# Algolzw/image-restoration-sde

Measured on AMD Instinct MI355X. Metric: restored images/sec at 256x256, 100-step IR-SDE reverse sampler, higher is better.
Workload: dtype f32; 1 GPU; IR-SDE deraining ConditionalUNet nf=64 depth=4, reverse_sde, batch=16/GPU 256x256, T=100 (BASELINE.json configs[1]); compute_dtype=fp32, global_batch=16

## Files before the change

### image_restoration_sde_amd/_lib.py

```python
import ctypes
import os
import subprocess
import threading

_HERE = os.path.dirname(os.path.abspath(__file__))
LIB_PATH = os.environ.get("IRSDE_LIB_PATH") or os.path.join(_HERE, "libirsde_hip.so")
CSRC = os.path.join(_HERE, "csrc")

MODE = {"sde": 0, "ode": 1, "posterior": 2, "dsde_sde": 3, "dsde_ode": 4}
COEF_STRIDE = 12
FLAG_KEEP_ACTIVATIONS = 1
FLAG_NAIVE_CONV = 2
FLAG_NO_WINOGRAD = 4
FLAG_NO_WINOGRAD_F43 = 8
FLAG_UNCOND_FULLATTN = 16
FLAG_BF16 = 32
FLAG_NAF_INTRO_SKIP = 64
FLAG_BF16_ACT = 128
FLAG_NO_FUSED_LN = 256
FLAG_NAF_LENS = 512
FLAG_FP16 = 1024
FLAG_NO_WINOGRAD_FUSED = 2048
FLAG_NO_FUSED_ATTN = 4096
FLAG_NO_NAF_CHAIN = 8192
FLAG_SPLIT_BF16X2 = 16384
FLAG_SPLIT_F16X2 = 32768
FLAG_NAF_STEREO = 65536
FLAG_NAF_UNCOND = 131072
FLAG_UNET_STEREO = 262144
FLAG_F16_ACT = 524288
FLAG_NO_WINO_POLY = 1048576
FLAG_SCAM_STREAM = 2097152
FLAG_NO_SPLIT3 = 4194304
SAMPLE_GRAPH = 1
SAMPLE_PROFILE = 2

SYMBOLS = [
    "irsde_last_error", "irsde_version", "irsde_create", "irsde_create_nafnet", "irsde_destroy", "irsde_num_weights",
    "irsde_weight_name", "irsde_weight_shape", "irsde_load_weight", "irsde_finalize_weights",
    "irsde_set_schedule", "irsde_unet_forward", "irsde_sample", "irsde_sde_step", "irsde_philox_normal",
    "irsde_get_profile", "irsde_debug_tap", "irsde_work_model", "irsde_debug_conv", "irsde_debug_conv_choice", "irsde_debug_conv_features", "irsde_plan_describe", "irsde_bench_conv", "irsde_op_profile", "irsde_debug_split_gemm", "irsde_bench_naf_chain", "irsde_debug_force_subbatches", "irsde_debug_force_chain_groups", "irsde_debug_force_wino_poly", "irsde_debug_force_split3", "irsde_debug_force_split3_blocks", "irsde_debug_scam", "irsde_debug_scam_full",
    "irsde_debug_scam_stream", "irsde_debug_scam_full_stream", "irsde_debug_force_scam_stream",
    "irsde_debug_naf_gate_sca", "irsde_debug_tlsc", "irsde_debug_ln_film", "irsde_debug_naf_lnconv", "irsde_debug_naf_chain", "irsde_debug_naf_chain_split_order",
    "irsde_debug_full_attention16",
    "irsde_eval_metrics", "irsde_tensor2img",
    "irsde_set_lens_info", "irsde_nafnet_set_local_pool", "irsde_create_latent_unet", "irsde_latent_shapes", "irsde_latent_encode", "irsde_latent_decode", "irsde_latent_hidden",
]


class IrsdeLibraryError(RuntimeError):
    pass


class IrsdeError(RuntimeError):
    pass


class Config(ctypes.Structure):
    _fields_ = [("in_nc", ctypes.c_int32), ("out_nc", ctypes.c_int32), ("nf", ctypes.c_int32),
                ("depth", ctypes.c_int32), ("device", ctypes.c_int32), ("flags", ctypes.c_int32)]


class NafConfig(ctypes.Structure):
    _fields_ = [("img_channel", ctypes.c_int32), ("width", ctypes.c_int32), ("middle_blk_num", ctypes.c_int32),
                ("n_enc", ctypes.c_int32), ("enc_blk_nums", ctypes.c_int32 * 8), ("n_dec", ctypes.c_int32),
                ("dec_blk_nums", ctypes.c_int32 * 8), ("device", ctypes.c_int32), ("flags", ctypes.c_int32)]


class LatentConfig(ctypes.Structure):
    _fields_ = [("in_ch", ctypes.c_int32), ("out_ch", ctypes.c_int32), ("ch", ctypes.c_int32), ("n_mult", ctypes.c_int32),
                ("ch_mult", ctypes.c_int32 * 8), ("embed_dim", ctypes.c_int32), ("device", ctypes.c_int32),
                ("flags", ctypes.c_int32)]


_lib = None
_lock = threading.Lock()


PROBES_LIB_PATH = os.path.join(_HERE, "libirsde_hip_probes.so")


def build_library(force=False, verbose=False, probes=True):
    if force:
        subprocess.run(["make", "-C", CSRC, "clean"], check=True, capture_output=not verbose)
    for extra in ([], ["PROBES=1"]) if probes else ([],):
        r = subprocess.run(["make", "-j8", "-C", CSRC] + extra, capture_output=True, text=True)
        if r.returncode != 0:
            raise IrsdeLibraryError("building libirsde_hip%s.so failed:\n" % ("_probes" if extra else "") + r.stdout + r.stderr)
        if verbose:
            print(r.stdout)
    return LIB_PATH


def _declare(lib):
    c = ctypes
    P = c.c_void_p
    lib.irsde_last_error.restype = c.c_char_p
    lib.irsde_last_error.argtypes = []
    lib.irsde_version.restype = c.c_int
    lib.irsde_create.argtypes = [c.POINTER(Config), c.POINTER(P)]
    lib.irsde_create_nafnet.argtypes = [c.POINTER(NafConfig), c.POINTER(P)]
    lib.irsde_destroy.argtypes = [P]
    lib.irsde_destroy.restype = None
    lib.irsde_num_weights.argtypes = [P]
    lib.irsde_weight_name.argtypes = [P, c.c_int]
    lib.irsde_weight_name.restype = c.c_char_p
    lib.irsde_weight_shape.argtypes = [P, c.c_int, c.POINTER(c.c_int64), c.POINTER(c.c_int)]
    lib.irsde_load_weight.argtypes = [P, c.c_char_p, P, c.POINTER(c.c_int64), c.c_int]
    lib.irsde_finalize_weights.argtypes = [P]
    lib.irsde_set_schedule.argtypes = [P, c.c_int, P]
    lib.irsde_unet_forward.argtypes = [P, P, P, c.POINTER(c.c_int64), c.c_int, c.c_int, c.c_int, c.c_int, P, P]
    lib.irsde_sample.argtypes = [P, c.c_int, P, P, P, c.c_uint64, c.c_uint64, c.c_int, c.c_int, c.c_int,
                                 c.c_int, c.c_int, P, P, c.c_int]
    lib.irsde_sde_step.argtypes = [c.c_int, c.c_int, P, P, P, P, P, c.c_uint64, c.c_uint64, c.c_int, c.c_int,
                                   c.c_int, c.c_int, P]
    lib.irsde_philox_normal.argtypes = [P, c.c_int, c.c_int, c.c_int, c.c_uint64, c.c_uint64, P]
    lib.irsde_get_profile.argtypes = [P, c.POINTER(c.c_double)]
    lib.irsde_debug_tap.argtypes = [P, c.c_char_p, P, c.POINTER(c.c_int64)]
    lib.irsde_work_model.argtypes = [P, c.c_int, c.c_int, c.c_int, c.POINTER(c.c_double)]
    lib.irsde_debug_conv.argtypes = [P, c.c_int, P, c.c_int, c.c_int, c.c_int, c.c_int, c.c_int, P, c.c_int, c.c_int,
                                     c.c_int, c.c_int, c.c_int, P, P, c.c_int, c.c_int, P, P, c.c_int, c.c_int, P]
    lib.irsde_debug_conv_choice.argtypes = [c.c_int] * 13 + [c.c_uint] + [c.c_int] * 4 + [c.POINTER(c.c_int), c.c_char_p, c.c_int]
    lib.irsde_debug_conv_features.argtypes = ([P, c.c_int, P, c.c_int] + [c.c_int] * 4 + [P] + [c.c_int] * 7 + [P] * 3 + [P, c.c_int, P, P, P, c.c_int] + [c.c_int] * 6 +
                                              [c.POINTER(c.c_int), P, c.c_char_p, c.c_int, P])
    lib.irsde_plan_describe.argtypes = [P, c.c_int, c.c_int, c.c_int, c.c_char_p, c.c_int]
    lib.irsde_op_profile.argtypes = [P, c.c_char_p, c.c_int]
    lib.irsde_bench_conv.argtypes = [c.c_int] * 11 + [c.POINTER(c.c_double)]
    lib.irsde_bench_naf_chain.argtypes = [c.c_int] * 4 + [c.POINTER(c.c_double)]
    lib.irsde_debug_force_subbatches.argtypes = [c.c_int]
    lib.irsde_debug_force_chain_groups.argtypes = [c.c_int]
    lib.irsde_debug_force_wino_poly.argtypes = [c.c_int]
    lib.irsde_debug_force_split3.argtypes = [c.c_int]
    lib.irsde_debug_force_split3_blocks.argtypes = [c.c_int]
    lib.irsde_debug_scam.argtypes = [P, c.c_int, c.c_int, c.c_int, c.c_int] + [P] * 12 + [P, P]
    lib.irsde_debug_scam_full.argtypes = [P, c.c_int, c.c_int, c.c_int, c.c_int] + [P] * 12 + [P, P]
    lib.irsde_debug_scam_stream.argtypes = [P, c.c_int, c.c_int, c.c_int, c.c_int] + [P] * 12 + [c.c_int, P, P]
    lib.irsde_debug_scam_full_stream.argtypes = [P, c.c_int, c.c_int, c.c_int, c.c_int] + [P] * 12 + [c.c_int, P, P]
    lib.irsde_debug_force_scam_stream.argtypes = [c.c_int]
    lib.irsde_debug_naf_gate_sca.argtypes = [P, c.c_int, c.c_int, c.c_int, c.c_int] + [P] * 8
    lib.irsde_debug_tlsc.argtypes = [P] + [c.c_int] * 6 + [P] * 4
    lib.irsde_debug_ln_film.argtypes = [P, c.c_int64, c.c_int, c.c_int64, P, P, P, c.c_int, P, P]
    lib.irsde_debug_naf_lnconv.argtypes = [c.c_int, P, c.c_int64, c.c_int, c.c_int, c.c_int64, P, P, P, c.c_int, P, P, P, c.c_int, P, P, P, P, P]
    lib.irsde_debug_naf_chain.argtypes = [P, P, c.c_int, c.c_int] + [P] * 16 + [P, c.c_int, c.c_int, P, c.c_int, c.c_int, c.c_int, P]
    lib.irsde_debug_naf_chain_split_order.argtypes = [c.c_int, c.c_int, c.POINTER(c.c_int), c.c_int64]
    lib.irsde_debug_full_attention16.argtypes = [P, c.c_int, c.c_int, P, P]
    lib.irsde_debug_split_gemm.argtypes = [P, P, P, c.c_int, c.c_int, c.c_int, c.c_int, c.c_int, P]
    lib.irsde_eval_metrics.argtypes = [P, P, c.c_int, c.c_int, c.c_int, c.c_int, c.c_int, c.POINTER(c.c_double), P]
    lib.irsde_tensor2img.argtypes = [P, P, c.c_int, c.c_int, c.c_int, c.c_int, P]
    lib.irsde_set_lens_info.argtypes = [P, c.POINTER(c.c_float), c.c_int]
    lib.irsde_nafnet_set_local_pool.argtypes = [P, c.c_int, c.c_int, c.c_int, c.c_int]
    lib.irsde_create_latent_unet.argtypes = [c.POINTER(LatentConfig), c.POINTER(P)]
    lib.irsde_latent_shapes.argtypes = [P, c.c_int, c.c_int, c.POINTER(c.c_int64), c.POINTER(c.c_int64), c.POINTER(c.c_int)]
    lib.irsde_latent_encode.argtypes = [P, P, c.c_int, c.c_int, c.c_int, P, c.POINTER(P), P]
    lib.irsde_latent_decode.argtypes = [P, P, c.POINTER(P), c.c_int, c.c_int, c.c_int, P, P]
    lib.irsde_latent_hidden.argtypes = [P, c.c_int, c.c_int, c.c_int, c.c_int, P, P]
    for name in SYMBOLS:
        getattr(lib, name)
    return lib


def lib():
    global _lib
    with _lock:
        if _lib is None:
            if not os.path.exists(LIB_PATH):
                raise IrsdeLibraryError(
                    "libirsde_hip.so not found at %s — build it with `python -c 'import __graft_entry__ as g; "
                    "g.build()'` or `make -C %s`. There is no CPU/PyTorch fallback for this path." % (LIB_PATH, CSRC))
            try:
                _lib = _declare(ctypes.CDLL(LIB_PATH))
            except OSError as ex:
                raise IrsdeLibraryError("failed to load %s: %s" % (LIB_PATH, ex)) from ex
        return _lib


_probes = None


def probes_lib():
    global _probes
    with _lock:
        if _probes is None:
            if not os.path.exists(PROBES_LIB_PATH):
                raise IrsdeLibraryError("libirsde_hip_probes.so not found at %s — build it with `make -C %s PROBES=1`" % (PROBES_LIB_PATH, CSRC))
            try:
                _probes = _declare(ctypes.CDLL(PROBES_LIB_PATH))
            except OSError as ex:
                raise IrsdeLibraryError("failed to load %s: %s" % (PROBES_LIB_PATH, ex)) from ex
        return _probes


def check(rc, L=None):
    if rc != 0:
        msg = (L or lib()).irsde_last_error()
        raise IrsdeError("libirsde_hip error %d: %s" % (rc, msg.decode() if msg else "?"))


def stream_ptr(torch_stream=None):
    import torch
    s = torch_stream if torch_stream is not None else torch.cuda.current_stream()
    return ctypes.c_void_p(s.cuda_stream)
```

### image_restoration_sde_amd/csrc/common.h

```cpp
#pragma once
#include <hip/hip_runtime.h>
#include <cstdint>
#include <cstdio>
#include <cstdlib>
#include <stdexcept>
#include <string>
#include <vector>
#include "split3_layout.h"

namespace irsde {

struct HipError : std::runtime_error {
    using std::runtime_error::runtime_error;
};
struct HipOutOfMemory : HipError {
    using HipError::HipError;
};

inline int tuning_env_int(const char* name, int dflt) {
    static const bool on = [] { const char* t = getenv("IRSDE_TUNING"); return t && atoi(t) == 1; }();
    if (!on) return dflt;
    const char* v = getenv(name);
    return v ? atoi(v) : dflt;
}

#define IRSDE_HIP_CHECK(expr)                                                                  \
    do {                                                                                       \
        hipError_t _e = (expr);                                                                \
        if (_e != hipSuccess) {                                                                \
            throw ::irsde::HipError(std::string(#expr) + " failed: " + hipGetErrorString(_e) + \
                                    " (" __FILE__ ":" + std::to_string(__LINE__) + ")");       \
        }                                                                                      \
    } while (0)

struct ConvParams {
    const float* in0 = nullptr;
    const float* in1 = nullptr;
    int C0 = 0, C1 = 0;
    int pix0 = 0, pix1 = 0;
    int Hin = 0, Win = 0;
    int in_shift = 0;
    const float* w = nullptr;
    const unsigned short* w_bf = nullptr;
    int f16 = 0;
    const unsigned short* w_pair = nullptr;
    float pair_scale = 1.f;
    int Cout = 0;
    int KH = 1, KW = 1, stride = 1, pad_y = 0, pad_x = 0;
    int B = 0, Ho = 0, Wo = 0;
    float* out = nullptr;
    int out_stride = 0;
    const float* bias = nullptr;
    const float* film = nullptr;
    int film_bstride = 0;
    int silu = 0;
    const float* res = nullptr;
    int res_stride = 0;
    int splits = 1;
    float* partial = nullptr;
    const float* zeros = nullptr;
    const float* ch_scale = nullptr;
    const float* in_scale = nullptr;
    int gate = 0;
    const float* gate_film = nullptr;
    int gate_film_bstride = 0;
    int shuffle = 0;
    int nz = 1;
    long long z_in = 0, z_w = 0, z_out = 0;
    int no_direct_epi = 0;
    int in_bf16 = 0, out_bf16 = 0;
    int in_f16 = 0, out_f16 = 0;
    const float* ln_g = nullptr;
    float ln_eps = 1e-5f;
};

struct WinoParams {
    const float* in0 = nullptr;
    const float* in1 = nullptr;
    int C0 = 0, C1 = 0, Hin = 0, Win = 0, in_shift = 0;
    int B = 0, TH = 0, TW = 0, T = 0;
    int tile = 2;
    float* V = nullptr;
    unsigned short* Vs = nullptr;
    int nplanes = 0;
    int v_f16 = 0;
    float v_scale = 1.f;
    int v_pairs = 0;
    int v_triples = 0;
    const float* M = nullptr;
    int Cout = 0;
    float* out = nullptr;
    int out_stride = 0;
    const float* bias = nullptr;
    const float* film = nullptr;
    int film_bstride = 0;
    int silu = 0;
    const float* res = nullptr;
    int res_stride = 0;
};
void launch_wino_input(const WinoParams& p, hipStream_t s);
struct WinoPolyParams {
    int up = 0;
    const float* in = nullptr;
    int C = 0, Hin = 0, Win = 0;
    int B = 0, TH = 0, TW = 0, T = 0;
    float* V = nullptr;
    unsigned short* Vs = nullptr;
    int thread_writer = 0;
    const float* M = nullptr;
    int Cout = 0, Ho = 0, Wo = 0;
    float* out = nullptr;
    int out_stride = 0;
    const float* bias = nullptr;
};
void launch_wino_poly_input(const WinoPolyParams& p, hipStream_t s);
void launch_wino_poly_output(const WinoPolyParams& p, hipStream_t s);
void wino_poly_transform_weights(const float* w_packed, int Cout, int Cin, float* U, int up);
struct SplitGemmArgs {
    const unsigned short* a = nullptr;
    const unsigned short* b = nullptr;
    float* out = nullptr;
    long long plA = 0, plB = 0, pA = 0, pB = 0, pO = 0;
    int M = 0, N = 0, K = 0, lda = 0, ldc = 0;
    float out_scale = 1.f;
    int n_inner = 1;
    int nblk_n = 0;
};
void gemm_split_global_init();
void launch_gemm_split_pairs(const SplitGemmArgs& a, int ncomp, hipStream_t s, int abl = 0, bool f16 = false);
void launch_split_pairs(const float* in, unsigned short* out, size_t rows, int K, hipStream_t s, bool f16 = false,
                        float scale = 1.0f);
struct Split3Launch {
    enum Abl { FULL = 0, NO_LOADS = 1, NO_MFMA = 3, NO_STORES = 4 };
    enum Tri { RULE, ON, OFF };
    Abl abl = FULL;
    Tri walk = RULE;
    Tri drain = RULE;
};
void launch_gemm_split_triples(const SplitGemmArgs& a, int ncomp, hipStream_t s, const Split3Launch& o = {});
void set_force_split3_blocks(int n);
bool gemm_split_triples_fits(long long M, long long N, long long K, long long ldc);
void launch_split_triples(const float* in, unsigned short* out, int ncomp, size_t rows, int K, hipStream_t s);
void launch_split_planes(const float* in, unsigned short* out, size_t n, size_t plane, int nplanes, hipStream_t s, bool f16 = false,
                         float scale = 1.0f);
void launch_wino_output(const WinoParams& p, hipStream_t s);
void wino_transform_weights(const float* w_packed, int Cout, int Cin, float* U, int tile);
bool wino_fused_eligible(const ConvParams& p);
void wino_fused_pack_weights(const float* U, int Cout, int Cin, float* Uf);
void launch_wino_fused(const ConvParams& p, const float* Uf, hipStream_t s, unsigned long long* dbg = nullptr, int dflags = 0);
int wino_fused_num_blocks(const ConvParams& p);
bool wino_fused64_eligible(const ConvParams& p);
void wino_fused64_pack_weights(const float* U, int Cout, int Cin, float* Uf);
void launch_wino_fused64(const ConvParams& p, const float* Uf, hipStream_t s, int variant = 0);
void wino_fused64_set_debug(unsigned long long* buf);
constexpr float kWinoFused64PairVScale = 0.0625f;
void launch_wino_fused64_split_weights(const float* Uf, unsigned short* out, size_t nfloats, float scale, hipStream_t s);
int wino_fused64_num_blocks(const ConvParams& p);
bool wino_fused64_xcd_nb(const ConvParams& p);
void wino_fused_global_init();
int device_cu_count();
bool wino_fused64t_eligible(const ConvParams& p);
long long wino_fused64t_num_items(const ConvParams& p);
void launch_wino_fused64t(const ConvParams& p, const float* Uf, hipStream_t s, int variant = 0);
void wino_fused64t_set_debug(unsigned long long* buf);
void wino_fused_t_global_init();
void naf_chain_global_init();
void naf_chain_set_debug(unsigned long long* buf);
bool naf_chain_shape_ok(int H, int W, int c);
size_t naf_chain_weight_halves(int nblocks);
size_t naf_chain_vec_floats(int nblocks);
void launch_naf_chain(const float* x, float* out, const unsigned short* w, const float* vecs, int nblocks, int B, const float* film, int film_bstride,
                      int film_off, const float* cam, int cam_bstride, int cam_off, hipStream_t s, int variant = 0);
std::vector<int> naf_chain_split_order(int nblocks, int G);
void naf_chain_build_split_weights(const unsigned short* w1, unsigned short* dst, int nblocks, int G, hipStream_t s);
size_t naf_chain_split_scratch_bytes(int B);
int naf_chain_split_groups(int B, int G);
void launch_naf_chain_split(const float* x, float* out, const unsigned short* wG, const float* vecs, int nblocks, int B, const float* film, int film_bstride,
                            int film_off, const float* cam, int cam_bstride, int cam_off, int G, void* scratch, hipStream_t s);
const unsigned* naf_chain_split_error_flag(const void* scratch, int B);
void naf_chain_split_reset(void* scratch, int B);
void naf_chain_set_sabotage(int on);
void attention_global_init();

double conv_flops(const ConvParams& p);
struct ConvTune {
    enum Tile { TILE_AUTO, TILE_128, TILE_256x128, TILE_256, TILE_128_ONE_PER_CU };
    enum Halo { HALO_AUTO, HALO_OFF, HALO_FORCE_512, HALO_FORCE_256 };
    enum ZLoop { ZLOOP_AUTO, ZLOOP_OFF, ZLOOP_ALL, ZLOOP_PAIRS, ZLOOP_FORCE_1X1 };
    bool rules_off = false;
    Tile tile = TILE_AUTO;
    bool no_buffer_desc = false;
    bool no_direct_epi = false;
    Halo halo = HALO_AUTO;
    ZLoop zloop = ZLOOP_AUTO;
};
struct ConvKnobs {
    int small_bn = 2, small_bn_f32 = 0;
    int pair_tile256 = 1, pair_inscale256 = 0;
    int no_bufa = 0;
    int zloop = -1, zloop_1x1 = -1;
    int zloop_maxnk = 32, zloop_minblk = 1024, zloop_deep = 1, zloop_ragged64 = 2048;
};
const ConvKnobs& conv_knobs_from_env();
struct ConvChoice {
    enum Family { PAIR, NARROW3, ZLOOP_BATCH, ZLOOP_1X1, HALO, IGEMM };
    enum Operand { OP_F32, OP_F32_BUF, OP_BF16, OP_F16 };
    enum Storage { ACT_F32, ACT_BF16, ACT_F16 };
    Family family = IGEMM;
    int BM = 0, BN = 0;
    Operand op = OP_F32;
    Storage act = ACT_F32;
    bool inscale = false;
    int zbatch = 0, zrows = 0;
    unsigned gx = 0, gy = 1, gz = 1;
    int threads = 0, lds = 0;
    int row = -1;
    std::string name() const;
    long long blocks() const { return (long long)gx * gy * gz; }
};
int conv_base_bn(int Cout);
void conv_validate(const ConvParams& p);
ConvChoice conv_choose(const ConvParams& p, const ConvTune& t, const ConvKnobs& k, int cu_count);
int conv_instance_count();
void launch_conv(const ConvParams& p, hipStream_t s, const ConvTune& t = {}, const ConvKnobs* knobs = nullptr, ConvChoice* chosen = nullptr);
void conv_global_init();
void conv_halo_global_init();
bool conv_halo_eligible(const ConvParams& p);
bool conv_halo2_wanted(const ConvParams& p, int force);
void launch_conv_halo(const ConvParams& p, hipStream_t s, int force_halo2 = 0);
void launch_fill_random(float* p, size_t n, unsigned seed, float scale, hipStream_t s);
__device__ __forceinline__ float silu_hw(const float v) {
    return v * __builtin_amdgcn_rcpf(1.0f + __builtin_amdgcn_exp2f(v * -1.44269504088896341f));
}

void launch_f32_to_bf16(const float* in, unsigned short* out, size_t n, hipStream_t s);
void launch_f32_to_f16(const float* in, unsigned short* out, size_t n, hipStream_t s);
void launch_bf16_to_f32(const unsigned short* in, float* out, size_t n, hipStream_t s);
void launch_f16_to_f32(const unsigned short* in, float* out, size_t n, hipStream_t s);
void launch_conv_naive(const ConvParams& p, hipStream_t s);

void launch_layernorm(const float* x, const float* g, const float* res, float* out, int64_t M, int C,
                      float eps, hipStream_t s, bool bf16 = false);
void launch_layernorm_film(const float* x, const float* g, const float* scale, const float* shift, int film_bstride,
                           int64_t pixels_per_image, float* out, int64_t M, int C, float eps, hipStream_t s,
                           bool f16 = false);
int dwgate_tiles(int H, int W, int c);
bool naf_lnconv_ok(int c, int Cout, long long M);
void launch_naf_pwconv(const float* x, const float* in_scale, int64_t pixels_per_image, const unsigned short* w16, const float* bias, const float* ch_scale,
                       const float* res, float* out, int64_t M, int c, int Cout, hipStream_t s, bool f16 = false);
void naf_lnconv_global_init();
void launch_naf_lnconv(const float* x, const float* g, const float* fscale, const float* fshift, int film_bstride, int64_t pixels_per_image,
                       const unsigned short* w16, const float* bias, float* out, int64_t M, int c, int Cout, int gate, const float* gate_film,
                       int gate_film_bstride, hipStream_t s, bool f16 = false);
void launch_dwconv_gate(const float* u, const float* w, const float* bias, float* out, float* partial, int B, int H, int W,
                        int c, hipStream_t s, bool f16 = false);
void launch_sca(const float* partial, int ntiles, const float* W, const float* bias, float* mean, float* s_out, int B,
                int c, int HW, hipStream_t s);
void launch_sca_mean(const float* partial, int ntiles, float* mean, int B, int c, int HW, hipStream_t s);
void tlsc_check_shape(int B, int h, int w, int c, int k1, int k2);
void launch_tlsc_pool(const float* gated, float* rowsum, float* pooled, int B, int h, int w, int c, int k1, int k2, hipStream_t s);
void launch_tlsc_scale(float* gated, const float* scale, int B, int h, int w, int c, int k1, int k2, hipStream_t s);
void launch_row_gate(const float* in, float* out, int rows, int h, hipStream_t s);

struct AttnWorkspace {
    float* pmax = nullptr;
    float* pctx = nullptr;
    float* psum = nullptr;
    float* ctx = nullptr;
    int nch = 0;
};
int attn_num_chunks(int N, int B);
void launch_linear_attention(const float* qkv, float* out, int B, int N, const AttnWorkspace& ws, hipStream_t s,
                             bool bf16 = false);

void launch_attention_kv_context(const float* xn, const float* wkv, int B, int N, int C, const AttnWorkspace& ws, hipStream_t s,
                                 const float* ln_g = nullptr, float ln_eps = 1e-5f, const unsigned short* wkv_pair = nullptr,
                                 float w_inv_scale = 1.f, int op16 = 0, bool act_bf16 = false);
void launch_attention_q_out(const float* q, float* out, int B, int N, const AttnWorkspace& ws, hipStream_t s);
void launch_attention_q_out_fused(const float* xn, const float* x, const float* wq, const float* wout, const float* bias,
                                  const float* g2, float* y, int B, int N, int C, float eps, const AttnWorkspace& ws, hipStream_t s,
                                  const float* ln_g = nullptr, const unsigned short* wq_pair = nullptr, const unsigned short* wout_pair = nullptr,
                                  float wq_inv = 1.f, float wout_inv = 1.f, int op16 = 0, bool act_bf16 = false);

void scam_check_shape(int H, int W, int c, bool any_width = false);
void launch_scam_prologue(const float* x, const float* g_l, const float* g_r, float* xs2, int B, int H, int W, int c, hipStream_t s);
void launch_scam_core(const float* qv, float* F, int B, int H, int W, int c, hipStream_t s);
void launch_scam_epilogue(const float* x, const float* F, const float* beta, const float* gamma, float* out, int B, int H, int W, int c, hipStream_t s);
void scam_pack_proj(const float* w1, const float* b1, const float* w2, const float* b2, int c, std::vector<float>& w, std::vector<float>& bias);
constexpr int kScamFullMaxW = 1024;
constexpr int kScamFullMaxC = 2048;
void scam_full_check_shape(int H, int W, int c, bool any_width = false);
void launch_scam_full_prologue(const float* x, const float* g_l, const float* g_r, float* x2, int B, int H, int W, int c, hipStream_t s);
void launch_scam_full_core(const float* qv, float* F, int B, int H, int W, int c, hipStream_t s);
void launch_scam_full_epilogue(float* x, const float* F, const float* beta, const float* gamma, int B, int H, int W, int c, hipStream_t s);
constexpr int kScamMaxWs = 512;
constexpr int kScamStreamMaxBlockW = 512;
bool scam_stream_block_ok(int block_w);
void launch_scam_stream_core(const float* qv, float* F, int B, int Hs, int Ws, int c, int block_w, hipStream_t s);
void launch_stereo_prep(const float* xt, const float* cond, float* x0, int B, int ic, int P, int H, int W, int Hp, int Wp, hipStream_t s);
void launch_stereo_pack_pred(const float* in, float* out, int B, int ic, int Hp, int Wp, int in_stride, int out_stride, hipStream_t s);
void launch_stereo_unet_prep(const float* xt, const float* cond, float* x0, int B, int ic, int P, int H, int W, int Hp, int Wp, hipStream_t s);
void launch_stereo_unet_pack_pred(const float* in, const float* xt, float* out, int B, int ic, int H, int W, int Hp, int Wp, int in_stride, int out_stride,
                                  hipStream_t s);

void launch_full_attention(const float* qkv, float* out, int B, int N, hipStream_t s);
void launch_full_attention16(const unsigned short* qkv, unsigned short* out, int B, int N, hipStream_t s);

void launch_prep_input(const float* xt, const float* cond, float* x0, int B, int in_nc, int H, int W, int Hp, int Wp,
                       hipStream_t s, int reflect = 1);

enum Act { ACT_NONE = 0, ACT_SILU = 1, ACT_GELU = 2 };
void launch_sinusoid(const float* tvals, const float* freqs, float* out, int rows, int half, hipStream_t s);
void launch_row_linear(const float* in, int in_stride, const float* W, const float* b, float* out, int out_stride,
                       int rows, int in_dim, int out_dim, int act_in, int act_out, hipStream_t s);

struct StepState {
    int t;
    int t_next;
    int pad0, pad1;
    float coef[12];
};
void launch_step_begin(StepState* st, const float* film_table, int film_row, float* film_cur,
                       const float* coef_table, hipStream_t s);
void launch_set_step(StepState* st, int t_next, hipStream_t s);

struct SampleCtl {
    int mode;
    int pad;
    const float* noise;
    long long noise_tstride;
    unsigned long long seed;
    unsigned long long image_offset;
};
void launch_set_ctl(SampleCtl* ctl, int mode, const float* noise, long long noise_tstride, unsigned long long seed,
                    unsigned long long image_offset, hipStream_t s);

void launch_unpack_pred(const float* pred, float* out, int B, int C, int H, int W, int Hp, int Wp, int stride, hipStream_t s);
void launch_add(const float* a, const float* b, float* out, size_t n, hipStream_t s);
void launch_nchw_to_nhwc_pad(const float* in, float* out, int B, int C, int H, int W, int Hp, int Wp, int Cp, int reflect,
                             hipStream_t s);
void launch_nhwc_to_nchw(const float* in, float* out, int B, int C, int H, int W, hipStream_t s, bool bf16 = false, bool f16 = false);

struct UpdateParams {
    float* x;
    const float* mu;
    const float* pred;
    int64_t sb, sc, sy, sx;
    const float* noise;
    int64_t noise_tstride;
    const StepState* st;
    const SampleCtl* ctl;
    int t_imm;
    float coef_imm[12];
    int mode;
    int B, C, H, W;
    uint64_t seed;
    uint64_t image_offset;
    int batch0;
};
void launch_sde_update(const UpdateParams& p, hipStream_t s);
void launch_philox_normal(float* out, int B, int CHW, int t, uint64_t seed, uint64_t image_offset, hipStream_t s);

void eval_metrics(const float* out, const float* gt, int B, int C, int H, int W, int crop, double* sums_host, hipStream_t s);
void tensor2img_u8(const float* in, unsigned char* out, int B, int C, int H, int W, hipStream_t s);

}
```

### image_restoration_sde_amd/csrc/engine_debug.hip

```cpp
#include "engine.h"
#include "../../include/irsde_hip_debug.h"

using namespace irsde;

namespace irsde {
namespace {

struct Scratch {
    hipStream_t s;
    std::vector<void*> bufs;
    explicit Scratch(hipStream_t s_) : s(s_) {}
    ~Scratch() {
        (void)hipStreamSynchronize(s);
        for (void* p : bufs) (void)hipFree(p);
    }
    Scratch(const Scratch&) = delete;
    Scratch& operator=(const Scratch&) = delete;
    template <class T> T* alloc(size_t n) {
        void* p = nullptr;
        IRSDE_HIP_CHECK(hipMalloc(&p, n * sizeof(T)));
        bufs.push_back(p);
        return static_cast<T*>(p);
    }
    float* upload(const float* host, size_t n) {
        float* d = alloc<float>(n);
        IRSDE_HIP_CHECK(hipMemcpy(d, host, n * sizeof(float), hipMemcpyHostToDevice));
        return d;
    }
    float* upload(const std::vector<float>& v) { return upload(v.data(), v.size()); }
};
struct OwnedStream {
    hipStream_t s = nullptr;
    explicit OwnedStream(unsigned flags) { IRSDE_HIP_CHECK(hipStreamCreateWithFlags(&s, flags)); }
    ~OwnedStream() { (void)hipStreamDestroy(s); }
    OwnedStream(const OwnedStream&) = delete;
    OwnedStream& operator=(const OwnedStream&) = delete;
};
struct EventPair {
    hipEvent_t e0 = nullptr, e1 = nullptr;
    EventPair() {
        IRSDE_HIP_CHECK(hipEventCreate(&e0));
        IRSDE_HIP_CHECK(hipEventCreate(&e1));
    }
    ~EventPair() {
        if (e0) (void)hipEventDestroy(e0);
        if (e1) (void)hipEventDestroy(e1);
    }
    EventPair(const EventPair&) = delete;
    EventPair& operator=(const EventPair&) = delete;
};
template <class Run>
double time_launches(hipStream_t s, int iters, Run&& run) {
    EventPair ev;
    IRSDE_HIP_CHECK(hipEventRecord(ev.e0, s));
    for (int i = 0; i < iters; ++i) run();
    IRSDE_HIP_CHECK(hipEventRecord(ev.e1, s));
    IRSDE_HIP_CHECK(hipStreamSynchronize(s));
    float ms = 0.f;
    IRSDE_HIP_CHECK(hipEventElapsedTime(&ms, ev.e0, ev.e1));
    return ms / iters;
}


ConvTune conv_tune_from_code(int code) {
    ConvTune t;
    t.rules_off = code != 0;
    switch (code) {
        case 3: t.tile = ConvTune::TILE_256x128; break;
        case 50: t.tile = ConvTune::TILE_256; break;
        case 5: t.tile = ConvTune::TILE_128_ONE_PER_CU; break;
        case 6: t.no_buffer_desc = true; break;
        case 7: t.no_direct_epi = true; break;
        case 60: t.tile = ConvTune::TILE_256; t.halo = ConvTune::HALO_OFF; break;
        case 61: t.tile = ConvTune::TILE_128; t.halo = ConvTune::HALO_OFF; break;
        case 64: t.halo = ConvTune::HALO_FORCE_512; break;
        case 65: t.halo = ConvTune::HALO_FORCE_256; break;
        case 70: t.zloop = ConvTune::ZLOOP_OFF; break;
        case 71: t.zloop = ConvTune::ZLOOP_ALL; break;
        case 72: t.zloop = ConvTune::ZLOOP_PAIRS; break;
        case 73: t.zloop = ConvTune::ZLOOP_FORCE_1X1; break;
        default: break;
    }
    return t;
}

Split3Launch split3_launch_twin(int twin, int abl = 0) {
    Split3Launch o;
    o.abl = static_cast<Split3Launch::Abl>(abl);
    o.walk = twin == 0 ? Split3Launch::RULE : twin == 1 ? Split3Launch::OFF : Split3Launch::ON;
    o.drain = twin == 0 ? Split3Launch::RULE : twin == 1 ? Split3Launch::OFF : Split3Launch::ON;
    return o;
}

enum class Operand { F32, BF16, F16 };

enum class ConvPath {
    Direct,
    Valu,
    WinoF2,
    WinoF4,
    Poly,
    PolyTriples,
    F4Triples,
    F4Pairs,
    DirectPair,
    Fused32,
    Fused64,
    Fused64Pair,
    Fused64T,
};
struct DebugConvRow {
    int code;
    ConvPath path;
    Operand op;
    bool act_bf16;
    int tune;
    int variant;
    bool up;
    bool thread_writer;
};
constexpr DebugConvRow direct(int code, Operand op, bool act_bf16, int tune) { return {code, ConvPath::Direct, op, act_bf16, tune, 0, false, false}; }
constexpr DebugConvRow on_path(int code, ConvPath path, Operand op = Operand::F32) { return {code, path, op, false, 0, 0, false, false}; }
constexpr DebugConvRow wino(int code, ConvPath path, int tune) { return {code, path, Operand::F32, false, tune, 0, false, false}; }
constexpr DebugConvRow poly(int code, ConvPath path, bool up, bool thread_writer = false) { return {code, path, Operand::F32, false, 0, 0, up, thread_writer}; }
constexpr DebugConvRow fused(int code, ConvPath path, int variant) { return {code, path, Operand::F32, false, 0, variant, false, false}; }
constexpr DebugConvRow kDebugConv[] = {
    direct(0, Operand::F32, false, 0),
    on_path(1, ConvPath::Valu),
    wino(2, ConvPath::WinoF2, 0), wino(12, ConvPath::WinoF2, 71), wino(22, ConvPath::WinoF2, 72),
    wino(3, ConvPath::WinoF4, 0), wino(13, ConvPath::WinoF4, 71), wino(23, ConvPath::WinoF4, 72),
    poly(24, ConvPath::Poly, false), poly(25, ConvPath::Poly, true),
    poly(26, ConvPath::PolyTriples, false), poly(27, ConvPath::PolyTriples, true), poly(28, ConvPath::PolyTriples, true, true),
    on_path(48, ConvPath::F4Triples),
    on_path(44, ConvPath::F4Pairs, Operand::F16), on_path(45, ConvPath::F4Pairs, Operand::BF16),
    on_path(46, ConvPath::DirectPair, Operand::F16), on_path(47, ConvPath::DirectPair, Operand::BF16),
    on_path(33, ConvPath::Fused32),
    fused(34, ConvPath::Fused64, 0), fused(36, ConvPath::Fused64, 64), fused(55, ConvPath::Fused64, 20),
    fused(35, ConvPath::Fused64Pair, 4), fused(37, ConvPath::Fused64Pair, 4 + 64), fused(56, ConvPath::Fused64Pair, 24),
    fused(62, ConvPath::Fused64T, 0), fused(63, ConvPath::Fused64T, 64),
    direct(4, Operand::BF16, false, 0), direct(160, Operand::BF16, false, 60), direct(161, Operand::BF16, false, 61), direct(162, Operand::BF16, false, 64),
    direct(163, Operand::BF16, false, 65),
    direct(5, Operand::F16, false, 0), direct(165, Operand::F16, false, 61), direct(166, Operand::F16, false, 64), direct(167, Operand::F16, false, 65),
    direct(204, Operand::BF16, true, 0), direct(260, Operand::BF16, true, 60), direct(261, Operand::BF16, true, 61), direct(262, Operand::BF16, true, 64),
    direct(263, Operand::BF16, true, 65),
    direct(100, Operand::F32, false, 0), direct(103, Operand::F32, false, 3), direct(105, Operand::F32, false, 5), direct(106, Operand::F32, false, 6),
    direct(107, Operand::F32, false, 7), direct(150, Operand::F32, false, 50), direct(170, Operand::F32, false, 70), direct(171, Operand::F32, false, 71),
    direct(172, Operand::F32, false, 72), direct(173, Operand::F32, false, 73),
};

enum class BenchKind {
    Conv,
    Fused32,
    Fused32Stamps,
    Wino3,
    Wino3Gemm,
    Fused64,
    Fused64Stamps,
    Fused64T,
    Fused64TStamps,
    PairGemm,
    TripleGemm,
};
struct BenchRow {
    int lo, hi;
    BenchKind kind;
    int arg;
    Operand op;
    bool pair;
    bool act_bf16;
};
constexpr BenchRow bench(int lo, int hi, BenchKind kind, int arg, Operand op = Operand::F32, bool pair = false, bool act_bf16 = false) {
    return {lo, hi, kind, arg, op, pair, act_bf16};
}
constexpr BenchRow kBenchConv[] = {
    bench(0, 0, BenchKind::Conv, 0), bench(3, 3, BenchKind::Conv, 3), bench(5, 7, BenchKind::Conv, 5), bench(50, 50, BenchKind::Conv, 50),
    bench(70, 73, BenchKind::Conv, 70),
    bench(60, 61, BenchKind::Conv, 60, Operand::BF16),
    bench(62, 62, BenchKind::Conv, 0, Operand::BF16),
    bench(63, 63, BenchKind::Conv, 0, Operand::BF16, false, true),
    bench(64, 65, BenchKind::Conv, 64, Operand::BF16),
    bench(66, 67, BenchKind::Conv, 64, Operand::BF16, false, true),
    bench(480, 480, BenchKind::Conv, 0, Operand::F16, true), bench(481, 481, BenchKind::Conv, 0, Operand::BF16, true),
    bench(482, 482, BenchKind::Conv, 61, Operand::F16, true),
    bench(80, 80, BenchKind::Fused32, 0),
    bench(83, 82 + 255, BenchKind::Fused32, 1),
    bench(82, 82, BenchKind::Fused32Stamps, 0),
    bench(81, 81, BenchKind::Wino3, 0), bench(421, 421, BenchKind::Wino3Gemm, 0),
    bench(430, 432, BenchKind::Fused64, 20),
    bench(434, 434, BenchKind::Fused64, 24, Operand::F16),
    bench(435, 435, BenchKind::Fused64Stamps, 25), bench(2004, 2004, BenchKind::Fused64Stamps, 25),
    bench(2001, 2002, BenchKind::Fused64Stamps, 28),
    bench(460, 462, BenchKind::Fused64T, 0),
    bench(467, 469, BenchKind::Fused64T, 6),
    bench(465, 465, BenchKind::Fused64TStamps, 5),
    bench(4650, 4653, BenchKind::Fused64TStamps, 12),
    bench(472, 476, BenchKind::PairGemm, 0),
    bench(490, 504, BenchKind::TripleGemm, 0),
};

template <class Row, size_t N, class Lo, class Hi>
constexpr bool codes_disjoint(const Row (&rows)[N], Lo lo, Hi hi) {
    for (size_t i = 0; i < N; ++i)
        for (size_t j = 0; j < N; ++j)
            if (i != j && lo(rows[i]) <= hi(rows[j]) && lo(rows[j]) <= hi(rows[i])) return false;
    return true;
}
constexpr int row_code(const DebugConvRow& r) { return r.code; }
constexpr int row_lo(const BenchRow& r) { return r.lo; }
constexpr int row_hi(const BenchRow& r) { return r.hi; }
static_assert(codes_disjoint(kDebugConv, row_code, row_code), "irsde_debug_conv: a selector code has two rows");
static_assert(codes_disjoint(kBenchConv, row_lo, row_hi), "irsde_bench_conv: a variant has two rows");

const DebugConvRow& debug_conv_lookup(int code) {
    for (const DebugConvRow& r : kDebugConv)
        if (r.code == code) return r;
    throw HipError("debug_conv: unknown selector code " + std::to_string(code));
}
struct BenchSel {
    const BenchRow& row;
    int arg;
};
BenchSel bench_conv_lookup(int code) {
    for (const BenchRow& r : kBenchConv)
        if (code >= r.lo && code <= r.hi) return {r, r.arg + (code - r.lo)};
    throw HipError("bench_conv: unknown variant " + std::to_string(code));
}

SplitGemmArgs split_gemm_args(const unsigned short* a, const unsigned short* b, float* C, int M, int N, int K, size_t pA, size_t pB) {
    SplitGemmArgs g;
    g.a = a; g.b = b; g.out = C;
    g.pA = (long long)pA; g.pB = (long long)pB; g.pO = (long long)M * N;
    g.M = M; g.N = N; g.K = K; g.lda = K; g.ldc = N;
    return g;
}
SplitGemmArgs split_triples(Scratch& mem, const float* A, const float* Bm, float* C, int M, int N, int K, int ncomp, hipStream_t s) {
    const size_t ea = split3_comp_elems((size_t)M, (size_t)K), eb = split3_comp_elems((size_t)N, (size_t)K);
    unsigned short *ta = mem.alloc<unsigned short>(ea * ncomp), *tb = mem.alloc<unsigned short>(eb * ncomp);
    launch_split_triples(A, ta, ncomp, (size_t)M, K, s);
    launch_split_triples(Bm, tb, ncomp, (size_t)N, K, s);
    return split_gemm_args(ta, tb, C, M, N, K, ea, eb);
}
SplitGemmArgs split_pairs(Scratch& mem, const float* A, const float* Bm, float* C, int M, int N, int K, int ncomp, hipStream_t s, bool f16 = false, float sa = 1.f,
                          float sb = 1.f) {
    unsigned short *pa = mem.alloc<unsigned short>((size_t)2 * ncomp * M * K), *pb = mem.alloc<unsigned short>((size_t)2 * ncomp * N * K);
    launch_split_pairs(A, pa, (size_t)ncomp * M, K, s, f16, sa);
    launch_split_pairs(Bm, pb, (size_t)ncomp * N, K, s, f16, sb);
    SplitGemmArgs g = split_gemm_args(pa, pb, C, M, N, K, (size_t)M * K, (size_t)N * K);
    g.out_scale = 1.0f / (sa * sb);
    return g;
}

void write_choice_line(const ConvChoice& c, char* out, int out_len) {
    snprintf(out, (size_t)out_len, "name=%s family=%d tile=%dx%d op=%d act=%d inscale=%d zbatch=%d zrows=%d grid=%ux%ux%u threads=%d lds=%d row=%d of %d",
             c.name().c_str(), (int)c.family, c.BM, c.BN, (int)c.op, (int)c.act, (int)c.inscale, c.zbatch, c.zrows, c.gx, c.gy, c.gz, c.threads, c.lds, c.row,
             conv_instance_count());
}

struct ScamHookArgs {
    const float* x;
    float* out;
    const float *norm_l_g, *norm_r_g, *l_proj1_w, *l_proj1_b, *r_proj1_w, *r_proj1_b, *l_proj2_w, *l_proj2_b, *r_proj2_w, *r_proj2_b, *beta, *gamma;
};
struct ScamHookDev {
    float *gl, *gr, *beta, *gamma;
    float *in2, *qv, *F;
    size_t vsz;
};
template <class ShapeCheck, class Prologue, class Tail>
void scam_hook(const ScamHookArgs& a, int B, int Hs, int Ws, int C, void* stream, ShapeCheck check_shape, Prologue prologue, Tail tail) {
    if (!a.x || !a.out || !a.norm_l_g || !a.norm_r_g || !a.l_proj1_w || !a.l_proj1_b || !a.r_proj1_w || !a.r_proj1_b || !a.l_proj2_w || !a.l_proj2_b ||
        !a.r_proj2_w || !a.r_proj2_b || !a.beta || !a.gamma)
        throw HipError("null argument");
    check_shape();
    hipStream_t s = reinterpret_cast<hipStream_t>(stream);
    conv_global_init();
    std::vector<float> wl, bl, wr, br;
    scam_pack_proj(a.l_proj1_w, a.l_proj1_b, a.l_proj2_w, a.l_proj2_b, C, wl, bl);
    scam_pack_proj(a.r_proj1_w, a.r_proj1_b, a.r_proj2_w, a.r_proj2_b, C, wr, br);
    Scratch mem(s);
    auto up = [&](const float* h, size_t n) {
        float* d = mem.alloc<float>(std::max<size_t>(n, 16));
        if (h) IRSDE_HIP_CHECK(hipMemcpy(d, h, n * 4, hipMemcpyHostToDevice));
        return d;
    };
    ScamHookDev d;
    d.gl = up(a.norm_l_g, C); d.gr = up(a.norm_r_g, C); d.beta = up(a.beta, C); d.gamma = up(a.gamma, C);
    float *dwl = up(wl.data(), wl.size()), *dbl = up(bl.data(), bl.size()), *dwr = up(wr.data(), wr.size()), *dbr = up(br.data(), br.size());
    d.vsz = (size_t)B * Hs * Ws * 2 * C;
    d.in2 = up(nullptr, 2 * d.vsz); d.qv = up(nullptr, 2 * d.vsz); d.F = up(nullptr, d.vsz);
    float* dz = up(nullptr, 256);
    IRSDE_HIP_CHECK(hipMemset(dz, 0, 1024));
    prologue(d, s);
    for (int v = 0; v < 2; ++v) {
        ConvParams p;
        p.in0 = d.in2 + v * d.vsz; p.C0 = 2 * C; p.pix0 = 2 * C;
        p.Hin = Hs; p.Win = Ws;
        p.w = v ? dwr : dwl; p.Cout = 2 * C; p.KH = p.KW = 1; p.stride = 1;
        p.B = B; p.Ho = Hs; p.Wo = Ws;
        p.out = d.qv + v * d.vsz; p.out_stride = 2 * C;
        p.bias = v ? dbr : dbl;
        p.zeros = dz;
        launch_conv(p, s);
    }
    tail(d, s);
    IRSDE_HIP_CHECK(hipStreamSynchronize(s));
}

}
}

extern "C" {

int irsde_debug_scam(const float* x, int B, int H, int W, int C, const float* norm_l_g, const float* norm_r_g, const float* l_proj1_w,
                     const float* l_proj1_b, const float* r_proj1_w, const float* r_proj1_b, const float* l_proj2_w, const float* l_proj2_b,
                     const float* r_proj2_w, const float* r_proj2_b, const float* beta, const float* gamma, float* out, void* stream) {
    return guard([&] {
        scam_hook(
            {x, out, norm_l_g, norm_r_g, l_proj1_w, l_proj1_b, r_proj1_w, r_proj1_b, l_proj2_w, l_proj2_b, r_proj2_w, r_proj2_b, beta, gamma}, B, H / 4, W / 4, C, stream,
            [&] {
                if (B < 1) throw HipError("debug_scam: bad shape");
                scam_check_shape(H, W, C);
            },
            [&](const ScamHookDev& d, hipStream_t s) { launch_scam_prologue(x, d.gl, d.gr, d.in2, B, H, W, C, s); },
            [&](const ScamHookDev& d, hipStream_t s) {
                launch_scam_core(d.qv, d.F, B, H, W, C, s);
                launch_scam_epilogue(x, d.F, d.beta, d.gamma, out, B, H, W, C, s);
            });
    });
}

int irsde_debug_scam_full(const float* x, int B, int H, int W, int C, const float* norm_l_g, const float* norm_r_g, const float* l_proj1_w,
                          const float* l_proj1_b, const float* r_proj1_w, const float* r_proj1_b, const float* l_proj2_w, const float* l_proj2_b,
                          const float* r_proj2_w, const float* r_proj2_b, const float* beta, const float* gamma, float* out, void* stream) {
    return guard([&] {
        scam_hook(
            {x, out, norm_l_g, norm_r_g, l_proj1_w, l_proj1_b, r_proj1_w, r_proj1_b, l_proj2_w, l_proj2_b, r_proj2_w, r_proj2_b, beta, gamma}, B, H, W, C, stream,
            [&] {
                if (B < 1 || (long long)B * H > 65535) throw HipError("debug_scam_full: bad shape");
                scam_full_check_shape(H, W, C);
            },
            [&](const ScamHookDev& d, hipStream_t s) { launch_scam_full_prologue(x, d.gl, d.gr, d.in2, B, H, W, C, s); },
            [&](const ScamHookDev& d, hipStream_t s) {
                launch_scam_full_core(d.qv, d.F, B, H, W, C, s);
                if (out != x) IRSDE_HIP_CHECK(hipMemcpyAsync(out, x, d.vsz * sizeof(float), hipMemcpyDeviceToDevice, s));
                launch_scam_full_epilogue(out, d.F, d.beta, d.gamma, B, H, W, C, s);
            });
    });
}

int irsde_debug_scam_stream(const float* x, int B, int H, int W, int C, const float* norm_l_g, const float* norm_r_g, const float* l_proj1_w,
                            const float* l_proj1_b, const float* r_proj1_w, const float* r_proj1_b, const float* l_proj2_w, const float* l_proj2_b,
                            const float* r_proj2_w, const float* r_proj2_b, const float* beta, const float* gamma, int block_w, float* out, void* stream) {
    return guard([&] {
        scam_hook(
            {x, out, norm_l_g, norm_r_g, l_proj1_w, l_proj1_b, r_proj1_w, r_proj1_b, l_proj2_w, l_proj2_b, r_proj2_w, r_proj2_b, beta, gamma}, B, H / 4, W / 4, C, stream,
            [&] {
                if (B < 1 || (long long)B * (H / 4) > 65535) throw HipError("debug_scam_stream: bad shape");
                if (block_w != 0 && !scam_stream_block_ok(block_w)) throw HipError("debug_scam_stream: block_w must be 0 or a multiple of 16 in [16, 512]");
                scam_check_shape(H, W, C, true);
            },
            [&](const ScamHookDev& d, hipStream_t s) { launch_scam_prologue(x, d.gl, d.gr, d.in2, B, H, W, C, s); },
            [&](const ScamHookDev& d, hipStream_t s) {
                launch_scam_stream_core(d.qv, d.F, B, H / 4, W / 4, C, block_w, s);
                launch_scam_epilogue(x, d.F, d.beta, d.gamma, out, B, H, W, C, s);
            });
    });
}

int irsde_debug_scam_full_stream(const float* x, int B, int H, int W, int C, const float* norm_l_g, const float* norm_r_g, const float* l_proj1_w,
                                 const float* l_proj1_b, const float* r_proj1_w, const float* r_proj1_b, const float* l_proj2_w, const float* l_proj2_b,
                                 const float* r_proj2_w, const float* r_proj2_b, const float* beta, const float* gamma, int block_w, float* out,
                                 void* stream) {
    return guard([&] {
        scam_hook(
            {x, out, norm_l_g, norm_r_g, l_proj1_w, l_proj1_b, r_proj1_w, r_proj1_b, l_proj2_w, l_proj2_b, r_proj2_w, r_proj2_b, beta, gamma}, B, H, W, C, stream,
            [&] {
                if (B < 1 || (long long)B * H > 65535) throw HipError("debug_scam_full_stream: bad shape");
                if (block_w != 0 && !scam_stream_block_ok(block_w)) throw HipError("debug_scam_full_stream: block_w must be 0 or a multiple of 16 in [16, 512]");
                scam_full_check_shape(H, W, C, true);
            },
            [&](const ScamHookDev& d, hipStream_t s) { launch_scam_full_prologue(x, d.gl, d.gr, d.in2, B, H, W, C, s); },
            [&](const ScamHookDev& d, hipStream_t s) {
                launch_scam_stream_core(d.qv, d.F, B, H, W, C, block_w, s);
                if (out != x) IRSDE_HIP_CHECK(hipMemcpyAsync(out, x, d.vsz * sizeof(float), hipMemcpyDeviceToDevice, s));
                launch_scam_full_epilogue(out, d.F, d.beta, d.gamma, B, H, W, C, s);
            });
    });
}

int irsde_debug_force_scam_stream(int block_w) {
    if (block_w != 0 && !scam_stream_block_ok(block_w)) return guard([&] { throw HipError("debug_force_scam_stream: block_w must be 0 or a multiple of 16 in [16, 512]"); });
    set_force_scam_stream(block_w);
    return IRSDE_OK;
}

int irsde_debug_naf_gate_sca(const float* u, int B, int H, int W, int c, const float* conv2_w, const float* conv2_b, const float* sca_w, const float* sca_b,
                             float* gated_out, float* mean_out, float* s_out, void* stream) {
    return guard([&] {
        if (!u || !conv2_w || !conv2_b || !sca_w || !sca_b || !gated_out || !s_out) throw HipError("null argument");
        if (B < 1 || B > 65535 || H < 1 || W < 1 || c < 4 || c % 4 || (long long)H * W >= (1ll << 31)) throw HipError("debug_naf_gate_sca: bad shape");
        hipStream_t s = reinterpret_cast<hipStream_t>(stream);
        conv_global_init();
        Scratch mem(s);
        float *dw = mem.upload(pack_dwconv_taps(conv2_w, 2 * c)), *db = mem.upload(conv2_b, (size_t)2 * c);
        float *dsw = mem.upload(sca_w, (size_t)c * c), *dsb = mem.upload(sca_b, c);
        const int nt = dwgate_tiles(H, W, c);
        float *partial = mem.alloc<float>((size_t)B * nt * c), *mean = mem.alloc<float>((size_t)B * c);
        launch_dwconv_gate(u, dw, db, gated_out, partial, B, H, W, c, s);
        launch_sca(partial, nt, dsw, dsb, mean, s_out, B, c, H * W, s);
        if (mean_out) launch_sca_mean(partial, nt, mean_out, B, c, H * W, s);
        IRSDE_HIP_CHECK(hipStreamSynchronize(s));
    });
}

int irsde_debug_tlsc(const float* g, int B, int h, int w, int c, int k1, int k2, float* pooled_out, const float* scale_map, float* scaled_out, void* stream) {
    return guard([&] {
        if (!g || !pooled_out || !scale_map || !scaled_out) throw HipError("null argument");
        tlsc_check_shape(B, h, w, c, k1, k2);
        hipStream_t s = reinterpret_cast<hipStream_t>(stream);
        conv_global_init();
        Scratch mem(s);
        float* rowsum = mem.alloc<float>((size_t)B * h * (w - k2 + 1) * c);
        launch_tlsc_pool(g, rowsum, pooled_out, B, h, w, c, k1, k2, s);
        IRSDE_HIP_CHECK(hipMemcpyAsync(scaled_out, g, (size_t)B * h * w * c * sizeof(float), hipMemcpyDeviceToDevice, s));
        launch_tlsc_scale(scaled_out, scale_map, B, h, w, c, k1, k2, s);
        IRSDE_HIP_CHECK(hipStreamSynchronize(s));
    });
}

int irsde_debug_ln_film(const float* x, long long M, int C, long long ppi, const float* g, const float* fscale, const float* fshift, int film_bstride,
                        float* out, void* stream) {
    return guard([&] {
        if (!x || !g || !fscale || !fshift || !out) throw HipError("null argument");
        if (M < 1 || ppi < 1 || C < 4 || C % 4 || C > 2048 || film_bstride < 0 || film_bstride % 4) throw HipError("debug_ln_film: bad shape");
        hipStream_t s = reinterpret_cast<hipStream_t>(stream);
        conv_global_init();
        Scratch mem(s);
        float* dg = mem.upload(g, C);
        launch_layernorm_film(x, dg, fscale, fshift, film_bstride, ppi, out, M, C, 1e-5f, s);
        IRSDE_HIP_CHECK(hipStreamSynchronize(s));
    });
}

int irsde_debug_full_attention16(const void* qkv_bf16, int B, int N, void* out_bf16, void* stream) {
    return guard([&] {
        if (!qkv_bf16 || !out_bf16) throw HipError("null argument");
        hipStream_t s = reinterpret_cast<hipStream_t>(stream);
        launch_full_attention16(static_cast<const unsigned short*>(qkv_bf16), static_cast<unsigned short*>(out_bf16), B, N, s);
        IRSDE_HIP_CHECK(hipStreamSynchronize(s));
    });
}

int irsde_debug_naf_lnconv(int mode, const float* x, long long M, int c, int Cout, long long ppi, const float* g, const float* fscale, const float* fshift,
                           int film_bstride, const float* w, const float* bias, const float* gate_film, int gate_film_bstride, const float* in_scale,
                           const float* ch_scale, const float* res, float* out, void* stream) {
    return guard([&] {
        if (mode < 0 || mode > 3) throw HipError("debug_naf_lnconv: mode must be 0 .. 3");
        if (!x || !w || !bias || !out) throw HipError("null argument");
        if (!naf_lnconv_ok(c, Cout, M) || ppi < 1) throw HipError("debug_naf_lnconv: bad shape");
        const bool ln = mode <= 1;
        if (ln && (!g || !fscale || !fshift || film_bstride < 0 || film_bstride % 4)) throw HipError("debug_naf_lnconv: modes 0 / 1 need g and the FiLM rows");
        if (mode == 1 && gate_film && gate_film_bstride < 0) throw HipError("debug_naf_lnconv: bad lens FiLM stride");
        if (!ln && (!ch_scale || !res || (mode == 2 && !in_scale))) throw HipError("debug_naf_lnconv: modes 2 / 3 need ch_scale and res, mode 2 in_scale");
        hipStream_t s = reinterpret_cast<hipStream_t>(stream);
        conv_global_init();
        std::vector<float> pw, pb;
        pack_conv_rows(w, bias, Cout, c, 1, 1, mode == 1 ? naf_gate_perm(Cout / 2) : std::vector<int>(), pw, pb);
        Scratch mem(s);
        float *dwf = mem.upload(pw), *dbias = mem.upload(pb);
        unsigned short* w16 = mem.alloc<unsigned short>(pw.size());
        launch_f32_to_f16(dwf, w16, pw.size(), s);
        if (ln) {
            float* dg = mem.upload(g, c);
            launch_naf_lnconv(x, dg, fscale, fshift, film_bstride, ppi, w16, dbias, out, M, c, Cout, mode, mode == 1 ? gate_film : nullptr,
                              mode == 1 && gate_film ? gate_film_bstride : 0, s);
        } else {
            float* dcs = mem.upload(ch_scale, Cout);
            launch_naf_pwconv(x, mode == 2 ? in_scale : nullptr, ppi, w16, dbias, dcs, res, out, M, c, Cout, s);
        }
        IRSDE_HIP_CHECK(hipStreamSynchronize(s));
    });
}

int irsde_debug_naf_chain(const float* x, float* out, int B, int nblocks, const float* norm1_g, const float* conv1_w, const float* conv1_b, const float* conv2_w,
                          const float* conv2_b, const float* sca_w, const float* sca_b, const float* conv3_w, const float* conv3_b, const float* beta,
                          const float* norm2_g, const float* conv4_w, const float* conv4_b, const float* conv5_w, const float* conv5_b, const float* gamma,
                          const float* film, int film_bstride, int film_off, const float* cam, int cam_bstride, int cam_off, int groups, void* stream) {
    return guard([&] {
        if (!x || !out || !norm1_g || !conv1_w || !conv1_b || !conv2_w || !conv2_b || !sca_w || !sca_b || !conv3_w || !conv3_b || !beta || !norm2_g || !conv4_w ||
            !conv4_b || !conv5_w || !conv5_b || !gamma || !film)
            throw HipError("null argument");
        if (B < 1 || B > 65535 || nblocks < 1 || nblocks > 64) throw HipError("debug_naf_chain: bad B or nblocks");
        if (groups != 1 && groups != 2 && groups != 4) throw HipError("debug_naf_chain: groups must be 1, 2 or 4");
        if (film_bstride < 0 || film_bstride % 4 || film_off < 0 || film_off % 4) throw HipError("debug_naf_chain: bad FiLM stride / offset");
        if (cam && (cam_bstride < 0 || cam_bstride % 4 || cam_off < 0 || cam_off % 4)) throw HipError("debug_naf_chain: bad lens FiLM stride / offset");
        hipStream_t s = reinterpret_cast<hipStream_t>(stream);
        conv_global_init();
        if (groups > 1 && naf_chain_split_groups(B, groups) > device_cu_count())
            throw HipError("debug_naf_chain: more work-groups than compute units (they must be co-resident)");
        constexpr size_t C = 512;
        std::vector<NafChainHostW> blocks(nblocks);
        for (int i = 0; i < nblocks; ++i) {
            NafChainHostW& b = blocks[i];
            const size_t k = (size_t)i;
            b.norm1_g = norm1_g + k * C; b.conv1_w = conv1_w + k * 2 * C * C; b.conv1_b = conv1_b + k * 2 * C;
            b.conv2_w = conv2_w + k * 18 * C; b.conv2_b = conv2_b + k * 2 * C;
            b.sca_w = sca_w + k * C * C; b.sca_b = sca_b + k * C;
            b.conv3_w = conv3_w + k * C * C; b.conv3_b = conv3_b + k * C; b.beta = beta + k * C;
            b.norm2_g = norm2_g + k * C; b.conv4_w = conv4_w + k * 2 * C * C; b.conv4_b = conv4_b + k * 2 * C;
            b.conv5_w = conv5_w + k * C * C; b.conv5_b = conv5_b + k * C; b.gamma = gamma + k * C;
        }
        std::vector<unsigned short> w;
        std::vector<float> vecs;
        pack_naf_chain_host(blocks, w, vecs);
        Scratch mem(s);
        unsigned short* dw = mem.alloc<unsigned short>(w.size());
        IRSDE_HIP_CHECK(hipMemcpy(dw, w.data(), w.size() * 2, hipMemcpyHostToDevice));
        float* dvec = mem.upload(vecs);
        if (groups == 1) {
            launch_naf_chain(x, out, dw, dvec, nblocks, B, film, film_bstride, film_off, cam, cam ? cam_bstride : 0, cam ? cam_off : 0, s, 0);
            IRSDE_HIP_CHECK(hipStreamSynchronize(s));
            return;
        }
        unsigned short* dwg = mem.alloc<unsigned short>(w.size());
        naf_chain_build_split_weights(dw, dwg, nblocks, groups, s);
        const size_t sb = naf_chain_split_scratch_bytes(B);
        char* dscratch = mem.alloc<char>(sb);
        IRSDE_HIP_CHECK(hipMemset(dscratch, 0, sb));
        launch_naf_chain_split(x, out, dwg, dvec, nblocks, B, film, film_bstride, film_off, cam, cam ? cam_bstride : 0, cam ? cam_off : 0, groups, dscratch, s);
        IRSDE_HIP_CHECK(hipStreamSynchronize(s));
        std::vector<unsigned> state((size_t)4 * B + 1);
        IRSDE_HIP_CHECK(hipMemcpy(state.data(), naf_chain_split_error_flag(dscratch, B) - 4 * B, state.size() * 4, hipMemcpyDeviceToHost));
        if (state[(size_t)4 * B]) throw HipError("debug_naf_chain: the split kernel's groups were not co-resident (spin timeout)");
        for (size_t i = 0; i < (size_t)4 * B; ++i)
            if (state[i]) throw HipError("debug_naf_chain: the split kernel left a barrier counter non-zero");
    });
}

int irsde_debug_naf_chain_split_order(int nblocks, int groups, int* order_out, long long n) {
    return guard([&] {
        if (!order_out || nblocks < 1 || nblocks > 64) throw HipError("debug_naf_chain_split_order: bad argument");
        const std::vector<int> order = naf_chain_split_order(nblocks, groups);
        if ((long long)order.size() != n) throw HipError("debug_naf_chain_split_order: the order has " + std::to_string(order.size()) + " entries");
        std::copy(order.begin(), order.end(), order_out);
    });
}

int irsde_debug_conv(const float* in0, int C0, const float* in1, int C1, int B, int Hin, int Win, int in_shift,
                     const float* w_oihw, int Cout, int KH, int KW, int stride, int pad, const float* bias,
                     const float* film, int film_bstride, int silu, const float* res, float* out, int naive,
                     int splits, void* stream) {
    return guard([&] {
        if (!in0 || !w_oihw || !out) throw HipError("null argument");
        const DebugConvRow& r = debug_conv_lookup(naive);
        hipStream_t s = reinterpret_cast<hipStream_t>(stream);
        conv_global_init();
        const int Cin = C0 + C1;
        std::vector<float> pk((size_t)Cout * KH * KW * Cin);
        for (int o = 0; o < Cout; ++o)
            for (int i = 0; i < Cin; ++i)
                for (int ky = 0; ky < KH; ++ky)
                    for (int kx = 0; kx < KW; ++kx)
                        pk[(((size_t)o * KH + ky) * KW + kx) * Cin + i] = w_oihw[(((size_t)o * Cin + i) * KH + ky) * KW + kx];
        Scratch mem(s);
        float* dw = mem.upload(pk);
        float* db = bias ? mem.upload(bias, Cout) : nullptr;
        ConvParams p;
        p.in0 = in0; p.C0 = C0; p.pix0 = C0; p.in1 = in1; p.C1 = C1; p.pix1 = C1;
        p.Hin = Hin; p.Win = Win; p.in_shift = in_shift;
        p.w = dw; p.Cout = Cout; p.KH = KH; p.KW = KW; p.stride = stride; p.pad_y = pad; p.pad_x = pad;
        p.B = B;
        p.Ho = ((Hin << in_shift) + 2 * pad - KH) / stride + 1;
        p.Wo = ((Win << in_shift) + 2 * pad - KW) / stride + 1;
        p.out = out; p.out_stride = Cout; p.bias = db; p.film = film; p.film_bstride = film_bstride; p.silu = silu;
        p.res = res; p.res_stride = Cout;
        float* dz = mem.alloc<float>(256);
        IRSDE_HIP_CHECK(hipMemset(dz, 0, 1024));
        p.zeros = dz;
        if (splits > 1 && r.path != ConvPath::Valu && r.path != ConvPath::WinoF2 && r.path != ConvPath::WinoF4) {
            p.splits = splits;
            p.partial = mem.alloc<float>((size_t)splits * B * p.Ho * p.Wo * Cout);
        }
        auto wino_weights = [&](int tile) {
            std::vector<float> U((size_t)(tile + 2) * (tile + 2) * Cout * Cin);
            wino_transform_weights(pk.data(), Cout, Cin, U.data(), tile);
            return U;
        };
        auto wino_tiles = [&](int tile) { return (long long)B * (p.Ho / tile) * (p.Wo / tile); };
        auto alloc_M = [&](int ncomp, long long T) { return mem.alloc<float>((size_t)ncomp * T * Cout); };
        auto poly_plan = [&](const char* refusal, float*& dU) {
            if (!(r.up ? wino_poly_up_shape(p) : wino_poly_down_shape(p)) || !wino_poly_eligible(p) || splits > 1) throw HipError(refusal);
            std::vector<float> U((size_t)100 * Cout * Cin);
            wino_poly_transform_weights(pk.data(), Cout, Cin, U.data(), r.up);
            dU = mem.upload(U);
            return make_wino_poly(p, dU, nullptr, nullptr);
        };
        switch (r.path) {
        case ConvPath::PolyTriples: {
            float* dU = nullptr;
            WinoPolyPlan wp = poly_plan("debug_conv: selectors 26 / 27 / 28 run what 24 / 25 run (single source, channels a multiple of 32, bias only)", dU);
            if (!gemm_split_triples_fits(wp.T, Cout, wp.K, Cout)) throw HipError("debug_conv: shape not eligible for the three-piece GEMM");
            unsigned short* dUt = mem.alloc<unsigned short>((size_t)wp.ncomp * split3_comp_elems((size_t)Cout, (size_t)wp.K));
            unsigned short* dVt = mem.alloc<unsigned short>((size_t)wp.ncomp * split3_comp_elems((size_t)wp.T, (size_t)wp.K));
            float* dM = alloc_M(wp.ncomp, wp.T);
            launch_split_triples(dU, dUt, wp.ncomp, (size_t)Cout, wp.K, s);
            wp = make_wino_poly(p, dU, nullptr, dM);
            const SplitGemmArgs sg = make_wino_poly_triples(wp, Cout, dUt, dVt, dM);
            wp.in.thread_writer = r.thread_writer;
            launch_wino_poly_input(wp.in, s);
            launch_gemm_split_triples(sg, wp.ncomp, s);
            launch_wino_poly_output(wp.out, s);
            break;
        }
        case ConvPath::Poly: {
            float* dU = nullptr;
            WinoPolyPlan wp = poly_plan(r.up ? "debug_conv: selector 25 runs a 3x3 stride-1 pad-1 convolution with in_shift = 1 (single source, channels a multiple of 32, bias only)"
                                             : "debug_conv: selector 24 runs a 4x4 stride-2 pad-1 convolution (single source, channels a multiple of 32, bias only)", dU);
            float* dV = mem.alloc<float>((size_t)wp.ncomp * wp.T * wp.K);
            wp = make_wino_poly(p, dU, dV, alloc_M(wp.ncomp, wp.T));
            launch_wino_poly_input(wp.in, s);
            launch_conv(wp.gemm, s);
            launch_wino_poly_output(wp.out, s);
            break;
        }
        case ConvPath::F4Triples: {
            if (!wino_shape_ok(p, 4) || Cin % 32) throw HipError("debug_conv: shape not eligible for the three-piece GEMM");
            const std::vector<float> U = wino_weights(4);
            const long long T = wino_tiles(4);
            if (!gemm_split_triples_fits(T, Cout, Cin, Cout)) throw HipError("debug_conv: shape not eligible for the three-piece GEMM");
            float* dU = mem.upload(U);
            unsigned short* dUt = mem.alloc<unsigned short>((size_t)36 * split3_comp_elems((size_t)Cout, (size_t)Cin));
            unsigned short* dVt = mem.alloc<unsigned short>((size_t)36 * split3_comp_elems((size_t)T, (size_t)Cin));
            launch_split_triples(dU, dUt, 36, (size_t)Cout, Cin, s);
            const WinoSplitPlan sp = make_wino_triples(p, dUt, dVt, alloc_M(36, T));
            launch_wino_input(sp.in, s);
            launch_gemm_split_triples(sp.gemm, 36, s);
            launch_wino_output(sp.out, s);
            break;
        }
        case ConvPath::F4Pairs: {
            const bool f16 = r.op == Operand::F16;
            if (!wino_shape_ok(p, 4) || Cin % 32) throw HipError("debug_conv: shape not eligible for the pair GEMM");
            std::vector<float> U = wino_weights(4);
            const float us = f16 ? pow2_scale_into_512(U.data(), U.size()) : 1.f;
            const long long T = wino_tiles(4);
            float* dU = mem.upload(U);
            unsigned short* dUp = mem.alloc<unsigned short>(2 * U.size());
            unsigned short* dVp = mem.alloc<unsigned short>((size_t)36 * T * Cin * 2);
            launch_split_pairs(dU, dUp, (size_t)36 * Cout, Cin, s, f16, us);
            const WinoSplitPlan sp = make_wino_pairs(p, dUp, dVp, alloc_M(36, T), f16, us);
            launch_wino_input(sp.in, s);
            launch_gemm_split_pairs(sp.gemm, 36, s, 0, f16);
            launch_wino_output(sp.out, s);
            break;
        }
        case ConvPath::Fused64Pair: {
            if (!wino_fused64_eligible(p)) throw HipError("debug_conv: shape not eligible for the fused Winograd kernel");
            std::vector<float> U = wino_weights(4), Uf(U.size());
            wino_fused64_pack_weights(U.data(), Cout, Cin, Uf.data());
            const float usc = pow2_scale_into_512(U.data(), U.size());
            float* dUf = mem.upload(Uf);
            unsigned short* dUp = mem.alloc<unsigned short>(2 * Uf.size());
            launch_wino_fused64_split_weights(dUf, dUp, Uf.size(), usc, s);
            p.pair_scale = 1.0f / (kWinoFused64PairVScale * usc);
            launch_wino_fused64(p, reinterpret_cast<const float*>(dUp), s, r.variant);
            break;
        }
        case ConvPath::Fused32:
        case ConvPath::Fused64:
        case ConvPath::Fused64T: {
            const bool f32k = r.path == ConvPath::Fused32;
            if (f32k ? !wino_fused_eligible(p) : !wino_fused64_eligible(p)) throw HipError("debug_conv: shape not eligible for the fused Winograd kernel");
            const std::vector<float> U = wino_weights(4);
            std::vector<float> Uf(U.size());
            if (f32k) wino_fused_pack_weights(U.data(), Cout, Cin, Uf.data());
            else wino_fused64_pack_weights(U.data(), Cout, Cin, Uf.data());
            float* dUf = mem.upload(Uf);
            if (r.path == ConvPath::Fused64T) {
                if (!wino_fused64t_eligible(p)) throw HipError("debug_conv: shape not eligible for the two-tile-group fused Winograd kernel");
                launch_wino_fused64t(p, dUf, s, r.variant);
            } else if (f32k) {
                launch_wino_fused(p, dUf, s);
            } else {
                launch_wino_fused64(p, dUf, s, r.variant);
            }
            break;
        }
        case ConvPath::WinoF2:
        case ConvPath::WinoF4: {
            const int tile = r.path == ConvPath::WinoF2 ? 2 : 4, ncomp = (tile + 2) * (tile + 2);
            if (!wino_shape_ok(p, tile)) throw HipError("debug_conv: shape not eligible for Winograd");
            const std::vector<float> U = wino_weights(tile);
            const long long T = wino_tiles(tile);
            float* dU = mem.upload(U);
            float* dV = mem.alloc<float>((size_t)ncomp * T * Cin);
            const WinoPlan wp = make_wino(p, dU, dV, alloc_M(ncomp, T), tile);
            launch_wino_input(wp.in, s);
            launch_conv(wp.gemm, s, conv_tune_from_code(r.tune));
            launch_wino_output(wp.out, s);
            break;
        }
        case ConvPath::DirectPair: {
            const bool f16 = r.op == Operand::F16;
            const float sc = f16 ? pow2_scale_into_512(pk.data(), pk.size()) : 1.f;
            unsigned short* dwp = mem.alloc<unsigned short>(2 * pk.size());
            launch_split_pairs(dw, dwp, (size_t)Cout, KH * KW * (C0 + C1), s, f16, sc);
            p.w_pair = dwp; p.pair_scale = 1.0f / sc; p.f16 = f16 ? 1 : 0;
            launch_conv(p, s);
            break;
        }
        case ConvPath::Valu:
            launch_conv_naive(p, s);
            break;
        case ConvPath::Direct: {
            unsigned short* ao = nullptr;
            if (r.op != Operand::F32) {
                unsigned short* d16 = mem.alloc<unsigned short>(pk.size());
                if (r.op == Operand::F16) launch_f32_to_f16(dw, d16, pk.size(), s);
                else launch_f32_to_bf16(dw, d16, pk.size(), s);
                p.w_bf = d16;
                p.f16 = r.op == Operand::F16 ? 1 : 0;
            }
            const size_t npix_in = (size_t)B * Hin * Win, nout = (size_t)B * p.Ho * p.Wo * Cout;
            if (r.act_bf16) {
                auto to_bf = [&](const float* src, size_t n) {
                    unsigned short* d = mem.alloc<unsigned short>(n + 32);
                    launch_f32_to_bf16(src, d, n, s);
                    return reinterpret_cast<const float*>(d);
                };
                p.in0 = to_bf(in0, npix_in * C0);
                if (in1) p.in1 = to_bf(in1, npix_in * C1);
                if (res) p.res = to_bf(res, nout);
                ao = mem.alloc<unsigned short>(nout + 32);
                p.out = reinterpret_cast<float*>(ao);
                p.in_bf16 = p.out_bf16 = 1;
            }
            launch_conv(p, s, conv_tune_from_code(r.tune));
            if (r.act_bf16) launch_bf16_to_f32(ao, out, nout, s);
            break;
        }
        }
        IRSDE_HIP_CHECK(hipStreamSynchronize(s));
    });
}

int irsde_debug_conv_choice(int B, int Hin, int Win, int C0, int C1, int Cout, int K, int stride, int pad, int in_shift, int operand, int storage, int pair,
                            unsigned features, int splits, int nz, int tune, int cu_count, const int* knobs, char* out, int out_len) {
    return guard([&] {
        if (!out || out_len < 1 || K < 1 || stride < 1 || cu_count < 1 || operand < 0 || operand > 2 || storage < 0 || storage > 2 || (pair && operand == 0))
            throw HipError("debug_conv_choice: bad argument");
        static const float dummy[4] = {};
        float* const some = const_cast<float*>(dummy);
        auto bit = [&](int i) { return (features >> i & 1u) ? some : nullptr; };
        ConvParams p;
        p.in0 = some; p.C0 = C0; p.pix0 = C0; p.in1 = C1 ? some : nullptr; p.C1 = C1; p.pix1 = C1;
        p.Hin = Hin; p.Win = Win; p.in_shift = in_shift;
        p.w = some; p.Cout = Cout; p.KH = K; p.KW = K; p.stride = stride; p.pad_y = pad; p.pad_x = pad;
        p.B = B;
        p.Ho = ((Hin << in_shift) + 2 * pad - K) / stride + 1;
        p.Wo = ((Win << in_shift) + 2 * pad - K) / stride + 1;
        p.out = some; p.out_stride = Cout; p.res_stride = Cout; p.zeros = some;
        p.bias = bit(0); p.film = bit(1); p.silu = bit(2) != nullptr; p.res = bit(3); p.in_scale = bit(4); p.ch_scale = bit(5);
        p.gate = bit(6) != nullptr; p.shuffle = bit(7) != nullptr; p.ln_g = bit(8);
        if (pair) p.w_pair = reinterpret_cast<const unsigned short*>(some);
        else if (operand) p.w_bf = reinterpret_cast<const unsigned short*>(some);
        p.f16 = operand == 2;
        p.in_bf16 = p.out_bf16 = storage == 1;
        p.in_f16 = p.out_f16 = storage == 2;
        p.nz = nz;
        if (splits > 1) { p.splits = splits; p.partial = some; }
        ConvKnobs k;
        static_assert(sizeof(ConvKnobs) == 11 * sizeof(int), "the hook's knob array is ConvKnobs, field by field");
        if (knobs) memcpy(&k, knobs, sizeof k);
        conv_validate(p);
        const ConvChoice c = conv_choose(p, conv_tune_from_code(tune), k, cu_count);
        const bool tabled = c.family != ConvChoice::NARROW3 && c.family != ConvChoice::HALO;
        if (tabled && c.row < 0) throw HipError("launch_conv: no kernel instance " + c.name());
        write_choice_line(c, out, out_len);
    });
}

int irsde_debug_conv_features(const float* in0, int C0, const float* in1, int C1, int B, int Hin, int Win, int in_shift, const float* w_oihw, int Cout, int K,
                              int stride, int pad, int operand, int storage, int pair, const float* bias, const float* ch_scale, const float* ln_g,
                              const float* film, int film_bstride, const float* res, const float* in_scale, const float* gate_film, int gate_film_bstride,
                              int silu, int gate, int shuffle, int nz, int splits, int tune, const int* knobs, float* out, char* choice, int choice_len,
                              void* stream) {
    return guard([&] {
        if (!in0 || !w_oihw || !out || !choice || choice_len < 1) throw HipError("null argument");
        if (B < 1 || Hin < 1 || Win < 1 || C0 < 1 || C1 < 0 || (C1 > 0) != (in1 != nullptr) || Cout < 1 || K < 1 || stride < 1 || pad < 0 || in_shift < 0 || in_shift > 1 ||
            operand < 0 || operand > 2 || storage < 0 || storage > 2 || (pair && operand == 0) || nz < 1 || splits < 1 || film_bstride < 0 || gate_film_bstride < 0)
            throw HipError("debug_conv_features: bad argument");
        if ((gate && shuffle) || (gate && (Cout % 4 || res)) || (shuffle && Cout % 4) || (gate_film && !gate) || ((gate || shuffle) && film))
            throw HipError("debug_conv_features: gate needs Cout % 4 == 0 and takes no residual, shuffle needs Cout % 4 == 0, gate_film goes with gate, film with neither");
        if (nz > 1 && (B != 1 || Hin != 1 || K != 1 || stride != 1 || pad || in_shift || C1 || storage))
            throw HipError("debug_conv_features: nz > 1 is a stack of 1x1 GEMMs: B = 1, Hin = 1, K = 1, one fp32 source");
        const int Ho = ((Hin << in_shift) + 2 * pad - K) / stride + 1, Wo = ((Win << in_shift) + 2 * pad - K) / stride + 1;
        if (Ho < 1 || Wo < 1) throw HipError("debug_conv_features: empty output");
        hipStream_t s = reinterpret_cast<hipStream_t>(stream);
        conv_global_init();
        const int Cin = C0 + C1;
        const std::vector<int> perm = gate ? naf_gate_perm(Cout / 2) : shuffle ? naf_shuffle_perm(Cout) : std::vector<int>();
        const size_t wz = (size_t)Cout * K * K * Cin;
        std::vector<float> pk(wz * nz), pb, one, oneb;
        for (int z = 0; z < nz; ++z) {
            pack_conv_rows(w_oihw + z * wz, z == 0 ? bias : nullptr, Cout, Cin, K, K, perm, one, z == 0 ? pb : oneb);
            std::copy(one.begin(), one.end(), pk.begin() + z * wz);
        }
        Scratch mem(s);
        float* dw = mem.upload(pk);
        ConvParams p;
        p.in0 = in0; p.C0 = C0; p.pix0 = C0; p.in1 = in1; p.C1 = C1; p.pix1 = C1;
        p.Hin = Hin; p.Win = Win; p.in_shift = in_shift;
        p.w = dw; p.Cout = Cout; p.KH = K; p.KW = K; p.stride = stride; p.pad_y = pad; p.pad_x = pad;
        p.B = B; p.Ho = Ho; p.Wo = Wo;
        const int ostride = gate ? Cout / 2 : shuffle ? Cout / 4 : Cout;
        const size_t npix_in = (size_t)B * Hin * Win * nz, M = (size_t)B * Ho * Wo, nout = M * nz * (gate ? Cout / 2 : Cout);
        p.out = out; p.out_stride = ostride; p.res = res; p.res_stride = ostride;
        if (bias) p.bias = mem.upload(pb);
        if (ch_scale) {
            std::vector<float> cs(Cout);
            for (int o = 0; o < Cout; ++o) cs[o] = ch_scale[perm.empty() ? o : perm[o]];
            p.ch_scale = mem.upload(cs);
        }
        if (ln_g) p.ln_g = mem.upload(ln_g, Cout);
        p.film = film; p.film_bstride = film_bstride; p.silu = silu; p.in_scale = in_scale;
        p.gate = gate ? 1 : 0; p.gate_film = gate_film; p.gate_film_bstride = gate_film ? gate_film_bstride : 0; p.shuffle = shuffle ? 1 : 0;
        p.nz = nz;
        if (nz > 1) { p.z_in = (long long)Win * C0; p.z_w = (long long)Cout * C0; p.z_out = (long long)Win * Cout; }
        float* dz = mem.alloc<float>(256);
        IRSDE_HIP_CHECK(hipMemset(dz, 0, 1024));
        p.zeros = dz;
        if (splits > 1) {
            p.splits = splits;
            p.partial = mem.alloc<float>((size_t)splits * M * Cout);
        }
        const bool f16 = operand == 2;
        unsigned short *w16 = nullptr, *a0 = nullptr, *a1 = nullptr, *ar = nullptr, *ao = nullptr;
        float wsc = 1.f;
        if (pair) {
            wsc = f16 ? pow2_scale_into_512(pk.data(), pk.size()) : 1.f;
            w16 = mem.alloc<unsigned short>(2 * pk.size());
            p.w_pair = w16; p.pair_scale = 1.0f / wsc;
        } else if (operand) {
            w16 = mem.alloc<unsigned short>(pk.size());
            p.w_bf = w16;
        }
        p.f16 = f16 ? 1 : 0;
        if (storage) {
            a0 = mem.alloc<unsigned short>(npix_in * C0);
            p.in0 = reinterpret_cast<const float*>(a0);
            if (in1) { a1 = mem.alloc<unsigned short>(npix_in * C1); p.in1 = reinterpret_cast<const float*>(a1); }
            if (res) { ar = mem.alloc<unsigned short>(nout); p.res = reinterpret_cast<const float*>(ar); }
            ao = mem.alloc<unsigned short>(nout);
            p.out = reinterpret_cast<float*>(ao);
            p.in_bf16 = p.out_bf16 = storage == 1;
            p.in_f16 = p.out_f16 = storage == 2;
        }
        ConvKnobs k;
        static_assert(sizeof(ConvKnobs) == 11 * sizeof(int), "the hook's knob array is ConvKnobs, field by field");
        if (knobs) memcpy(&k, knobs, sizeof k);
        conv_validate(p);
        auto narrow = [&](const float* src, unsigned short* dst, size_t n) {
            if (storage == 2) launch_f32_to_f16(src, dst, n, s);
            else launch_f32_to_bf16(src, dst, n, s);
        };
        if (pair) launch_split_pairs(dw, w16, (size_t)Cout * nz, K * K * Cin, s, f16, wsc);
        else if (operand == 2) launch_f32_to_f16(dw, w16, pk.size(), s);
        else if (operand == 1) launch_f32_to_bf16(dw, w16, pk.size(), s);
        if (storage) {
            narrow(in0, a0, npix_in * C0);
            if (in1) narrow(in1, a1, npix_in * C1);
            if (res) narrow(res, ar, nout);
            IRSDE_HIP_CHECK(hipMemsetAsync(ao, 0xFF, nout * 2, s));
        }
        ConvChoice c;
        launch_conv(p, s, conv_tune_from_code(tune), knobs ? &k : nullptr, &c);
        if (storage == 2) launch_f16_to_f32(ao, out, nout, s);
        else if (storage == 1) launch_bf16_to_f32(ao, out, nout, s);
        IRSDE_HIP_CHECK(hipStreamSynchronize(s));
        write_choice_line(c, choice, choice_len);
    });
}

int irsde_debug_split_gemm(const float* A, const float* Bm, float* C, int M, int N, int K, int ncomp, int nplanes, void* stream) {
    return guard([&] {
        const int twin3 = nplanes == 43 ? 0 : nplanes == 45 ? 1 : nplanes == 47 ? 2 : -1;
        if (twin3 < 0 && nplanes != 42 && nplanes != 44) throw HipError("debug_split_gemm: nplanes must be 42, 43, 44, 45 or 47");
        hipStream_t s = reinterpret_cast<hipStream_t>(stream);
        conv_global_init();
        Scratch mem(s);
        if (twin3 >= 0) {
            if (!gemm_split_triples_fits(M, N, K, N)) throw HipError("debug_split_gemm: shape not eligible for the three-piece GEMM");
            launch_gemm_split_triples(split_triples(mem, A, Bm, C, M, N, K, ncomp, s), ncomp, s, split3_launch_twin(twin3));
        } else {
            const bool f16 = nplanes == 44;
            launch_gemm_split_pairs(split_pairs(mem, A, Bm, C, M, N, K, ncomp, s, f16, f16 ? 1.0f / 16.0f : 1.f, f16 ? 64.0f : 1.f), ncomp, s, 0, f16);
        }
        IRSDE_HIP_CHECK(hipStreamSynchronize(s));
    });
}

int irsde_debug_force_chain_groups(int g) {
    set_force_chain_groups(g == 1 || g == 2 || g == 4 ? g : 0);
    return IRSDE_OK;
}

int irsde_debug_force_split3(int mode) {
    set_force_split3(mode >= 0 && mode <= 2 ? mode : -1);
    return IRSDE_OK;
}

int irsde_debug_force_split3_blocks(int n) {
    if (n >= 0 && n < 8) return guard([&] { throw HipError("debug_force_split3_blocks: n must be at least 8 (one block per XCD), or negative for the default"); });
    set_force_split3_blocks(n);
    return IRSDE_OK;
}

int irsde_debug_force_wino_poly(int mode) {
    set_force_wino_poly(mode >= 0 && mode <= 2 ? mode : -1);
    return IRSDE_OK;
}

int irsde_debug_force_subbatches(int n) {
    set_force_subbatches(n < 0 ? 0 : n);
    return IRSDE_OK;
}

int irsde_bench_naf_chain(int variant, int nblocks, int B, int iters, double* ms_out) {
    return guard([&] {
        if (!ms_out || nblocks < 1 || nblocks > 64 || B < 1 || iters < 1) throw HipError("bench_naf_chain: bad argument");
        const int G = variant == 22 ? 2 : (variant == 24 || variant == 25 || variant == 26) ? 4 : 1;
#ifdef IRSDE_PROBES
        if (variant != 0 && variant != 1 && variant != 11 && G == 1) throw HipError("bench_naf_chain: bad variant");
#else
        if (variant != 0 && variant != 1 && G == 1) throw HipError("bench_naf_chain: variant 11 is a measurement twin (make PROBES=1)");
#endif
        conv_global_init();
        OwnedStream stream(hipStreamDefault);
        hipStream_t s = stream.s;
        Scratch mem(s);
        const size_t nx = (size_t)B * 64 * 512, nw = naf_chain_weight_halves(nblocks), nv = naf_chain_vec_floats(nblocks);
        float *dx = mem.alloc<float>(nx), *dout = mem.alloc<float>(nx), *dvec = mem.alloc<float>(nv), *dfilm = mem.alloc<float>((size_t)nblocks * 2048);
        unsigned short* dw = mem.alloc<unsigned short>(nw);
        const size_t chunk = (size_t)64 << 20;
        float* dwf = mem.alloc<float>(chunk);
        launch_fill_random(dx, nx, 1, 1.0f, s);
        launch_fill_random(dvec, nv, 2, 0.1f, s);
        launch_fill_random(dfilm, (size_t)nblocks * 2048, 3, 0.1f, s);
        for (size_t o = 0; o < nw; o += chunk) {
            const size_t n = std::min(chunk, nw - o);
            launch_fill_random(dwf, n, 4 + (unsigned)(o / chunk), 0.04f, s);
            launch_f32_to_f16(dwf, dw + o, n, s);
        }
        unsigned short* dwg = nullptr;
        void* dscratch = nullptr;
        if (G > 1) {
            IRSDE_HIP_CHECK(hipStreamSynchronize(s));
            dwg = mem.alloc<unsigned short>(nw);
            naf_chain_build_split_weights(dw, dwg, nblocks, G, s);
            dscratch = mem.alloc<char>(naf_chain_split_scratch_bytes(B));
            IRSDE_HIP_CHECK(hipMemset(dscratch, 0, naf_chain_split_scratch_bytes(B)));
        }
        auto run = [&]() {
            if (G > 1) launch_naf_chain_split(dx, dout, dwg, dvec, nblocks, B, dfilm, 0, 0, nullptr, 0, 0, G, dscratch, s);
            else launch_naf_chain(dx, dout, dw, dvec, nblocks, B, dfilm, 0, 0, nullptr, 0, 0, s, variant == 11 ? 1 : variant);
        };
        if (variant == 26) {
#ifdef IRSDE_PROBES
            naf_chain_set_sabotage(1);
#else
            throw HipError("bench_naf_chain: variant 26 is a PROBES-build test");
#endif
        }
        struct SabotageOff { ~SabotageOff() { naf_chain_set_sabotage(0); } } sabotage_off;
        run();
        if (variant == 25) {
#ifdef IRSDE_PROBES
            const int ng = naf_chain_split_groups(B, 4);
            unsigned long long* dd = mem.alloc<unsigned long long>((size_t)ng * 8 * 16);
            IRSDE_HIP_CHECK(hipMemsetAsync(dd, 0, (size_t)ng * 8 * 16 * 8, s));
            naf_chain_set_debug(dd);
            run();
            IRSDE_HIP_CHECK(hipStreamSynchronize(s));
            naf_chain_set_debug(nullptr);
            std::vector<unsigned long long> hd((size_t)ng * 8 * 16);
            IRSDE_HIP_CHECK(hipMemcpy(hd.data(), dd, hd.size() * 8, hipMemcpyDeviceToHost));
            double acc[16] = {0};
            double nwv = 0;
            for (size_t w = 0; w < (size_t)ng * 8; ++w) {
                if (!hd[w * 16 + 15]) continue;
                for (int k = 0; k < 16; ++k) acc[k] += (double)hd[w * 16 + k];
                nwv += 1;
            }
            static const char* names[12] = {"norm1 (incl. residual-stream fetch)", "conv1 GEMM passes", "depthwise 3x3 + gate + pool", "gated fetch behind barrier (pool)", "sca.1 GEMM", "conv3 GEMM + residual", "norm2 (incl. residual-stream fetch)", "conv4 GEMM + gate", "conv5 GEMM + residual", "scale-vector / gated fetch (sca, conv4)", "group barriers (6 per block)", "publishing (gated slice, residual slice)"};
            printf("naf_chain stamps, 4 groups per image: %d blocks, B=%d; shader cycles per wave and block (mean over %.0f waves)\n", nblocks, B, nwv);
            for (int k = 0; k < 12; ++k) printf("  %-42s %9.0f\n", names[k], acc[k] / nwv / nblocks);
            printf("  %-42s %9.0f\n", "whole kernel / blocks", acc[15] / nwv / nblocks);
            fflush(stdout);
#else
            throw HipError("bench_naf_chain: variant 25 is a measurement twin (make PROBES=1)");
#endif
        }
        if (variant == 11) {
            unsigned long long* dd = mem.alloc<unsigned long long>((size_t)B * 8 * 16);
            IRSDE_HIP_CHECK(hipMemsetAsync(dd, 0, (size_t)B * 8 * 16 * 8, s));
            naf_chain_set_debug(dd);
            launch_naf_chain(dx, dout, dw, dvec, nblocks, B, dfilm, 0, 0, nullptr, 0, 0, s, 11);
            IRSDE_HIP_CHECK(hipStreamSynchronize(s));
            naf_chain_set_debug(nullptr);
            std::vector<unsigned long long> hd((size_t)B * 8 * 16);
            IRSDE_HIP_CHECK(hipMemcpy(hd.data(), dd, hd.size() * 8, hipMemcpyDeviceToHost));
            double acc[16] = {0};
            for (size_t i = 0; i < hd.size(); ++i) acc[i % 16] += (double)hd[i];
            const double nwv = (double)B * 8, nb = nblocks;
            static const char* names[10] = {"norm1", "conv1 GEMM passes", "depthwise 3x3 + gate + pool", "barrier (pool)", "sca.1 GEMM", "conv3 GEMM + residual", "norm2", "conv4 GEMM + gate", "conv5 GEMM + residual", "barriers (sca, conv4)"};
            printf("naf_chain stamps: %d blocks, B=%d; shader cycles per wave and block (mean over %d waves); MFMA floor per wave: conv1 / conv4 512 x 16, conv3 / conv5 256 x 16, sca 64 x 16\n", nblocks, B, B * 8);
            for (int k = 0; k < 10; ++k) printf("  %-30s %9.0f\n", names[k], acc[k] / nwv / nb);
            printf("  %-30s %9.0f\n", "whole kernel / blocks", acc[15] / nwv / nb);
            fflush(stdout);
        }
        *ms_out = time_launches(s, iters, run);
        if (G > 1) {
            unsigned flag = 0;
            IRSDE_HIP_CHECK(hipMemcpy(&flag, naf_chain_split_error_flag(dscratch, B), 4, hipMemcpyDeviceToHost));
            if (flag) throw HipError("bench_naf_chain: the split kernel's groups were not co-resident (spin timeout)");
        }
    });
}

int irsde_bench_conv(int variant, int B, int H, int W, int Cin, int Cout, int K, int stride, int up, int epi, int iters,
                     double* ms_out) {
    return guard([&] {
        if (!ms_out || iters < 1) throw HipError("bad argument");
        const BenchSel sel = bench_conv_lookup(variant);
        const BenchRow& r = sel.row;
        const BenchKind kind = r.kind;
        const int arg = sel.arg;
        conv_global_init();
        OwnedStream stream(hipStreamNonBlocking);
        hipStream_t s = stream.s;
        Scratch mem(s);
        ConvParams p;
        p.B = B; p.Hin = H; p.Win = W; p.in_shift = up; p.C0 = Cin; p.pix0 = Cin;
        p.Cout = Cout; p.KH = K; p.KW = K; p.stride = stride; p.pad_y = p.pad_x = (K == 4 ? 1 : K / 2);
        p.Ho = ((H << up) + 2 * p.pad_y - K) / stride + 1;
        p.Wo = ((W << up) + 2 * p.pad_x - K) / stride + 1;
        const size_t nin = (size_t)B * H * W * Cin, nw = (size_t)Cout * K * K * Cin, nout = (size_t)B * p.Ho * p.Wo * Cout;
        float *din = mem.alloc<float>(nin), *dw = mem.alloc<float>(nw), *dout = mem.alloc<float>(nout), *dres = mem.alloc<float>(nout);
        float* dfilm = mem.alloc<float>((size_t)2 * Cout + 256);
        float* dz = dfilm + 2 * Cout;
        IRSDE_HIP_CHECK(hipMemset(dz, 0, 1024));
        p.zeros = dz;
        launch_fill_random(din, nin, 1, 1.0f, s);
        launch_fill_random(dw, nw, 2, 1.0f / sqrtf((float)(K * K * Cin)), s);
        launch_fill_random(dres, nout, 3, 1.0f, s);
        launch_fill_random(dfilm, (size_t)2 * Cout, 4, 0.3f, s);
        p.in0 = din; p.w = dw; p.out = dout; p.out_stride = Cout;
        if (kind == BenchKind::Conv && r.op == Operand::BF16 && !r.pair) {
            unsigned short* dbf = mem.alloc<unsigned short>(nw);
            launch_f32_to_bf16(dw, dbf, nw, s);
            p.w_bf = dbf;
        }
        if (epi == 1) { p.film = dfilm; p.silu = 1; }
        if (epi == 2) { p.silu = 1; p.res = dres; p.res_stride = Cout; }
        if (r.act_bf16) {
            unsigned short* dabf = mem.alloc<unsigned short>(nin);
            launch_f32_to_bf16(din, dabf, nin, s);
            launch_f32_to_bf16(dout, reinterpret_cast<unsigned short*>(dres), nout / 2, s);
            p.in0 = reinterpret_cast<const float*>(dabf);
            p.in_bf16 = 1; p.out_bf16 = 1;
        }
        if (r.pair) {
            const bool f16 = r.op == Operand::F16;
            unsigned short* dwp = mem.alloc<unsigned short>(2 * nw);
            launch_split_pairs(dw, dwp, (size_t)Cout, K * K * Cin, s, f16, 64.0f);
            p.w_pair = dwp; p.pair_scale = 1.0f / 64.0f; p.f16 = f16 ? 1 : 0;
        }
        if (kind == BenchKind::TripleGemm || kind == BenchKind::PairGemm) {
            if (K != 3 || stride != 1 || !wino_shape_ok(p, 4)) throw HipError("bench_conv: Winograd variants need an eligible 3x3 stride-1 layer");
            const long long T = (long long)B * (p.Ho / 4) * (p.Wo / 4);
            const bool triples = kind == BenchKind::TripleGemm;
            if (triples && !gemm_split_triples_fits(T, Cout, Cin, Cout)) throw HipError("bench_conv: shape not eligible for the three-piece GEMM");
            float *vf = mem.alloc<float>((size_t)36 * T * Cin), *uf = mem.alloc<float>((size_t)36 * Cout * Cin), *mo = mem.alloc<float>((size_t)36 * T * Cout);
            launch_fill_random(vf, (size_t)36 * T * Cin, 7, 1.0f, s);
            launch_fill_random(uf, (size_t)36 * Cout * Cin, 8, 0.05f, s);
            const SplitGemmArgs g = triples ? split_triples(mem, vf, uf, mo, (int)T, Cout, Cin, 36, s) : split_pairs(mem, vf, uf, mo, (int)T, Cout, Cin, 36, s);
            const Split3Launch twin = split3_launch_twin(arg / 5, arg % 5);
            auto gemms = [&] {
                if (triples) launch_gemm_split_triples(g, 36, s, twin);
                else launch_gemm_split_pairs(g, 36, s, arg);
            };
            for (int i = 0; i < 2; ++i) gemms();
            *ms_out = time_launches(s, iters, gemms);
            return;
        }
        float* dU = nullptr;
        WinoPlan wp{};
        if (kind == BenchKind::Fused32Stamps) {
            dU = mem.alloc<float>((size_t)36 * nw / 9);
            launch_fill_random(dU, (size_t)36 * nw / 9, 5, 1.0f / sqrtf((float)(9 * Cin)), s);
            const int nb = wino_fused_num_blocks(p);
            unsigned long long* dd = mem.alloc<unsigned long long>((size_t)nb * 128);
            launch_wino_fused(p, dU, s);
            IRSDE_HIP_CHECK(hipMemsetAsync(dd, 0, (size_t)nb * 128 * 8, s));
            launch_wino_fused(p, dU, s, dd);
            IRSDE_HIP_CHECK(hipStreamSynchronize(s));
            std::vector<unsigned long long> hd((size_t)nb * 128);
            IRSDE_HIP_CHECK(hipMemcpy(hd.data(), dd, hd.size() * 8, hipMemcpyDeviceToHost));
            double ph[2][4] = {{0, 0, 0, 0}, {0, 0, 0, 0}};
            unsigned long long rt_min = ~0ull, rt_max = 0;
            for (int bi = 0; bi < nb; ++bi)
                for (int w = 0; w < 8; ++w) {
                    const unsigned long long* t = &hd[((size_t)bi * 8 + w) * 16];
                    for (int k = 0; k < 4; ++k) ph[w >= 4][k] += (double)(t[k + 1] - t[k]) / ((double)nb * 4);
                    rt_min = std::min(rt_min, t[7]);
                    rt_max = std::max(rt_max, t[7]);
                }
            printf("wino_fused timeline B=%d %dx%d Cin=%d Cout=%d: %d blocks, block starts span %.1f us\n", B, p.Ho, p.Wo, Cin, Cout, nb,
                   (double)(rt_max - rt_min) / 100.0);
            printf("  MFMA waves     (shader cycles): start->V[0] ready %.0f | K loop %.0f | acc->LDS+barrier %.0f | epilogue %.0f\n", ph[0][0],
                   ph[0][1], ph[0][2], ph[0][3]);
            printf("  producer waves (shader cycles): start->chunk 0 done %.0f | K loop rest %.0f | wait MFMA+acc %.0f | epilogue %.0f\n",
                   ph[1][0], ph[1][1], ph[1][2], ph[1][3]);
            fflush(stdout);
            *ms_out = 0.0;
            return;
        }
        if (kind != BenchKind::Conv) {
            const bool three_launch = kind == BenchKind::Wino3 || kind == BenchKind::Wino3Gemm;
            if (K != 3 || stride != 1) throw HipError("bench_conv: Winograd variants need a 3x3 stride-1 layer");
            dU = mem.alloc<float>((size_t)36 * nw / 9);
            launch_fill_random(dU, (size_t)36 * nw / 9, 5, 1.0f / sqrtf((float)(9 * Cin)), s);
            if (!three_launch && !wino_fused_eligible(p)) throw HipError("bench_conv: shape not eligible for the fused Winograd kernel");
            if (kind != BenchKind::Fused32 && kind != BenchKind::Wino3 && !wino_fused64_eligible(p))
                throw HipError("bench_conv: shape not eligible for the 64-cout fused Winograd kernel");
            if (kind == BenchKind::Fused64 && r.op == Operand::F16) {
                float* dUp = mem.alloc<float>((size_t)36 * nw / 9);
                launch_wino_fused64_split_weights(dU, reinterpret_cast<unsigned short*>(dUp), (size_t)36 * nw / 9, 256.0f, s);
                dU = dUp;
                p.pair_scale = 1.0f / (kWinoFused64PairVScale * 256.0f);
            }
            if (three_launch) {
                if (!wino_shape_ok(p, 4)) throw HipError("bench_conv: shape not eligible for Winograd F(4x4,3x3)");
                const long long T = (long long)B * (p.Ho / 4) * (p.Wo / 4);
                float* dV = mem.alloc<float>((size_t)36 * T * Cin);
                float* dM = mem.alloc<float>((size_t)36 * T * Cout);
                wp = make_wino(p, dU, dV, dM, 4);
                if (kind == BenchKind::Wino3Gemm) launch_wino_input(wp.in, s);
            }
        }
        if (kind == BenchKind::Fused64TStamps) {
            if (!wino_fused64t_eligible(p)) throw HipError("bench_conv: shape not eligible for the two-tile-group fused Winograd kernel");
            const int nbp = 256;
            unsigned long long* dd = mem.alloc<unsigned long long>((size_t)nbp * 64);
            launch_wino_fused64t(p, dU, s, 0);
            IRSDE_HIP_CHECK(hipMemsetAsync(dd, 0, (size_t)nbp * 64 * 8, s));
            wino_fused64t_set_debug(dd);
            launch_wino_fused64t(p, dU, s, arg);
            IRSDE_HIP_CHECK(hipStreamSynchronize(s));
            wino_fused64t_set_debug(nullptr);
            std::vector<unsigned long long> hd((size_t)nbp * 64);
            IRSDE_HIP_CHECK(hipMemcpy(hd.data(), dd, hd.size() * 8, hipMemcpyDeviceToHost));
            double a5[8] = {0, 0, 0, 0, 0, 0, 0, 0};
            int nwv = 0;
            for (int bi = 0; bi < nbp; ++bi)
                for (int w = 0; w < 8; ++w) {
                    const unsigned long long* t = &hd[((size_t)bi * 8 + w) * 8];
                    if (!t[3]) continue;
                    for (int k = 0; k < 8; ++k) a5[k] += (double)t[k];
                    nwv++;
                }
            const int nst = Cin / 16;
            const double items = a5[4] / std::max(nwv, 1), chunks = items * nst;
            printf("wino4_fused64t stamps B=%d %dx%d Cin=%d Cout=%d: %.1f items x %d chunks of 16 channels per block; shader cycles per wave (mean over %d waves)\n", B, p.Ho, p.Wo, Cin,
                   Cout, items, nst, nwv);
            printf("  kernel %.0f = K loops incl. transform slices %.0f (%.0f per chunk; MFMA floor per SIMD 9216) + chunk barrier waits %.0f (%.0f per chunk) + epilogue, exchange, first-chunk transform %.0f (%.0f per item)\n",
                   a5[3] / nwv, a5[0] / nwv, a5[0] / nwv / chunks, a5[1] / nwv, a5[1] / nwv / chunks, (a5[2] + a5[5] + a5[6] + a5[7]) / nwv, (a5[2] + a5[5] + a5[6] + a5[7]) / nwv / items);
            printf("  per item: first stage + exchange writes + ring %.0f | exchange barriers + reads %.0f | second stage, stores, gathers %.0f | zero, first-chunk transform, barrier %.0f\n",
                   a5[5] / nwv / items, a5[6] / nwv / items, a5[7] / nwv / items, a5[2] / nwv / items);
            fflush(stdout);
            *ms_out = 0.0;
            return;
        }
        if (kind == BenchKind::Fused64Stamps) {
            const int nbp = 256;
            unsigned long long* dd = mem.alloc<unsigned long long>((size_t)nbp * 64);
            launch_wino_fused64(p, dU, s, 20);
            IRSDE_HIP_CHECK(hipMemsetAsync(dd, 0, (size_t)nbp * 64 * 8, s));
            wino_fused64_set_debug(dd);
            launch_wino_fused64(p, dU, s, arg);
            IRSDE_HIP_CHECK(hipStreamSynchronize(s));
            wino_fused64_set_debug(nullptr);
            std::vector<unsigned long long> hd((size_t)nbp * 64);
            IRSDE_HIP_CHECK(hipMemcpy(hd.data(), dd, hd.size() * 8, hipMemcpyDeviceToHost));
            double acc[2][5] = {{0, 0, 0, 0, 0}, {0, 0, 0, 0, 0}};
            int nw[2] = {0, 0};
            for (int bi = 0; bi < nbp; ++bi)
                for (int w = 0; w < 8; ++w) {
                    const unsigned long long* t = &hd[((size_t)bi * 8 + w) * 8];
                    if (!t[3]) continue;
                    for (int k = 0; k < 5; ++k) acc[w >= 4][k] += (double)t[k];
                    nw[w >= 4]++;
                }
            const int nchk = Cin / 32;
            const double items = acc[0][4] / std::max(nw[0], 1), chunks = acc[1][4] / std::max(nw[1], 1);
            printf("wino4_fused64p stamps B=%d %dx%d Cin=%d Cout=%d: %.1f items x %d chunks per block; shader cycles per wave (mean over %d + %d waves)\n", B, p.Ho, p.Wo,
                   Cin, Cout, items, nchk, nw[0], nw[1]);
            printf("  MFMA waves    : kernel %.0f = K-loop compute %.0f (%.0f per chunk; MFMA floor 9216) + barrier wait %.0f (%.0f per chunk) + epilogue %.0f (%.0f per item)\n",
                   acc[0][3] / nw[0], acc[0][0] / nw[0], acc[0][0] / nw[0] / (items * nchk), acc[0][1] / nw[0], acc[0][1] / nw[0] / (items * nchk), acc[0][2] / nw[0],
                   acc[0][2] / nw[0] / items);
            printf("  producer waves: kernel %.0f = load issue %.0f (%.0f per chunk) + data wait, transform, LDS writes %.0f (%.0f per chunk) + barrier wait %.0f (%.0f per chunk)\n",
                   acc[1][3] / nw[1], acc[1][0] / nw[1], acc[1][0] / nw[1] / chunks, acc[1][1] / nw[1], acc[1][1] / nw[1] / chunks, acc[1][2] / nw[1], acc[1][2] / nw[1] / chunks);
            fflush(stdout);
            *ms_out = 0.0;
            return;
        }
        const ConvTune tune = kind == BenchKind::Conv ? conv_tune_from_code(arg) : ConvTune{};
        auto run = [&] {
            switch (kind) {
            case BenchKind::Fused32: launch_wino_fused(p, dU, s, nullptr, arg); break;
            case BenchKind::Fused64T: launch_wino_fused64t(p, dU, s, arg); break;
            case BenchKind::Fused64: launch_wino_fused64(p, dU, s, arg); break;
            case BenchKind::Wino3:
                launch_wino_input(wp.in, s);
                launch_conv(wp.gemm, s);
                launch_wino_output(wp.out, s);
                break;
            case BenchKind::Wino3Gemm: launch_conv(wp.gemm, s); break;
            default: launch_conv(p, s, tune); break;
            }
        };
        for (int i = 0; i < 2; ++i) run();
        *ms_out = time_launches(s, iters, run);
    });
}

}
```

### image_restoration_sde_amd/csrc/gemm_split.hip

```cpp
#include "common.h"
#include <algorithm>
#include <atomic>
#include <type_traits>

namespace irsde {

typedef float floatx16 __attribute__((ext_vector_type(16)));
typedef __bf16 bf16x8 __attribute__((ext_vector_type(8)));
typedef _Float16 f16x8 __attribute__((ext_vector_type(8)));
typedef unsigned uintx4 __attribute__((ext_vector_type(4)));

namespace {

constexpr int SG_BK = 32;

#define IRSDE_GLDS16(GPTR, LPTR) \
    __builtin_amdgcn_global_load_lds((const __attribute__((address_space(1))) void*)(GPTR), (__attribute__((address_space(3))) void*)(LPTR), 16, 0, 0)

template <int ABL = 0, bool F16 = false>
__global__ __launch_bounds__(512, 2) void gemm_split2i_kernel(const SplitGemmArgs g) {
    using frag_t = typename std::conditional<F16, f16x8, bf16x8>::type;
    constexpr int TM = 4, TN = 2, WN = 4, BM = 256, BN = 256;
    constexpr int A_STAGE = BM * 128, STAGE = (BM + BN) * 128;
    extern __shared__ __attribute__((aligned(16))) char lds[];
    const int tid = threadIdx.x, lane = tid & 63;
    const int wave = __builtin_amdgcn_readfirstlane(tid >> 6);
    const int wm = wave / WN, wn = wave % WN;
    const int l31 = lane & 31, h = lane >> 5;
    const int mtiles = (g.M + BM - 1) / BM;
    const int units = mtiles * g.n_inner;
    const int xcd = blockIdx.x & 7, jx = blockIdx.x >> 3;
    const int ulo = (int)((long long)xcd * units / 8), uhi = (int)((long long)(xcd + 1) * units / 8);
    const int unit = ulo + jx / g.nblk_n;
    if (unit >= uhi) return;
    const int nblk = jx % g.nblk_n;
    const int plane0 = unit / mtiles, mblk = unit - plane0 * mtiles;
    const int m0 = mblk * BM, n0 = nblk * BN;
    const int nk = g.K / SG_BK;
    const int steps = nk;
    const unsigned rowb = (unsigned)nk * 128u;

    unsigned a_voff[4], b_voff[4];
#pragma unroll
    for (int ps = 0; ps < 4; ++ps) {
        const int row = (ps * 8 + wave) * 8 + (lane >> 3);
        const unsigned pc = (unsigned)((lane & 7) ^ ((row >> 1) & 7)) * 16u;
        int m = m0 + row;
        m = m < g.M ? m : g.M - 1;
        a_voff[ps] = (unsigned)m * rowb + pc;
        int n = n0 + row;
        n = n < g.N ? n : g.N - 1;
        b_voff[ps] = (unsigned)n * rowb + pc;
    }
    const char* abase = reinterpret_cast<const char*>(g.a);
    const char* bbase = reinterpret_cast<const char*>(g.b);
    const long long pA2 = g.pA * 4, pB2 = g.pB * 4;
    int kb = 0;
    const char* acomp = abase + (long long)plane0 * pA2;
    const char* bcomp = bbase + (long long)plane0 * pB2;
    auto issue_loads = [&](int buf) {
        char* la = lds + buf * STAGE + wave * 1024;
        const char* ga = acomp + kb * 128;
        const char* gb = bcomp + kb * 128;
#pragma unroll
        for (int ps = 0; ps < 4; ++ps) IRSDE_GLDS16(ga + a_voff[ps], la + ps * 8192);
#pragma unroll
        for (int ps = 0; ps < 4; ++ps) IRSDE_GLDS16(gb + b_voff[ps], la + A_STAGE + ps * 8192);
    };

    auto issue_loads_part = [&](int buf, int part) {
        char* la = lds + buf * STAGE + wave * 1024;
        const char* ga = acomp + kb * 128;
        const char* gb = bcomp + kb * 128;
        if (part == 0) {
            IRSDE_GLDS16(ga + a_voff[0], la);
            IRSDE_GLDS16(ga + a_voff[1], la + 8192);
            IRSDE_GLDS16(ga + a_voff[2], la + 2 * 8192);
        } else if (part == 1) {
            IRSDE_GLDS16(ga + a_voff[3], la + 3 * 8192);
            IRSDE_GLDS16(gb + b_voff[0], la + A_STAGE);
            IRSDE_GLDS16(gb + b_voff[1], la + A_STAGE + 8192);
        } else {
            IRSDE_GLDS16(gb + b_voff[2], la + A_STAGE + 2 * 8192);
            IRSDE_GLDS16(gb + b_voff[3], la + A_STAGE + 3 * 8192);
        }
    };

    floatx16 acc[TM][TN];
#pragma unroll
    for (int i = 0; i < TM; ++i)
#pragma unroll
        for (int j = 0; j < TN; ++j)
#pragma unroll
            for (int r = 0; r < 16; ++r) acc[i][j][r] = 0.f;

    issue_loads(0);
    __syncthreads();

    const int wm_s = wm, wn_s = wn;
    unsigned o_voff[16];
#pragma unroll
    for (int r = 0; r < 16; ++r) o_voff[r] = (unsigned)(((r & 3) + 8 * (r >> 2) + 4 * h) * g.ldc + l31) * 4u;
    auto flush = [&](int fi) {
        const int rowb_ = m0 + wm_s * TM * 32, colb = n0 + wn_s * TN * 32;
        float* ob = g.out + (long long)(plane0 + fi) * g.pO + (long long)rowb_ * g.ldc;
        const int rows = g.M - rowb_;
        const unsigned nrec = rows <= 0 ? 0u : (unsigned)(rows < TM * 32 ? rows : TM * 32) * (unsigned)g.ldc * 4u;
        const __amdgpu_buffer_rsrc_t ro = __builtin_amdgcn_make_buffer_rsrc(ob, 0, nrec, 0x00020000);
#pragma unroll
        for (int i = 0; i < TM; ++i)
#pragma unroll
            for (int j = 0; j < TN; ++j) {
                const int colu = colb + j * 32;
                if (colu + l31 < g.N && (ABL != 4 || acc[i][j][0] == 1.2345e30f)) {
                    const int soff = (i * 32 * g.ldc + colu) * 4;
#pragma unroll
                    for (int r = 0; r < 16; ++r) {
                        const float v = F16 ? acc[i][j][r] * g.out_scale : acc[i][j][r];
                        __builtin_amdgcn_raw_buffer_store_b32(__builtin_bit_cast(unsigned, v), ro, (int)o_voff[r], soff, ABL == 5 ? 2 : 0);
                    }
                }
#pragma unroll
                for (int r = 0; r < 16; ++r) acc[i][j][r] = 0.f;
            }
    };
    const int swz = (l31 >> 1) & 7;
    int fr_off[2][2];
#pragma unroll
    for (int p = 0; p < 2; ++p)
#pragma unroll
        for (int sb = 0; sb < 2; ++sb) fr_off[p][sb] = l31 * 128 + (((p * 4 + sb * 2 + h) ^ swz) * 16);
    for (int st = 0; st < steps; ++st) {
        const int buf = st & 1;
        const bool more = st + 1 < steps;
        if (more) ++kb;
        const char* a = lds + buf * STAGE + wm * TM * 32 * 128;
        const char* b = lds + buf * STAGE + A_STAGE + wn * TN * 32 * 128;
        frag_t fa[2][2][TM], fb[2][2][TN];
#pragma unroll
        for (int sb = 0; sb < 2; ++sb)
#pragma unroll
            for (int p = 0; p < 2; ++p) {
#pragma unroll
                for (int i = 0; i < TM; ++i) fa[sb][p][i] = *reinterpret_cast<const frag_t*>(a + i * 32 * 128 + fr_off[p][sb]);
#pragma unroll
                for (int j = 0; j < TN; ++j) fb[sb][p][j] = *reinterpret_cast<const frag_t*>(b + j * 32 * 128 + fr_off[p][sb]);
            }
        __builtin_amdgcn_sched_barrier(0);
#pragma unroll
        for (int sb = 0; sb < 2; ++sb)
#pragma unroll
            for (int pr = 0; pr < 3; ++pr) {
#pragma unroll
                for (int i = 0; i < TM; ++i)
#pragma unroll
                    for (int j = 0; j < TN; ++j)
                        if (ABL != 3) {
                            if constexpr (F16) acc[i][j] = __builtin_amdgcn_mfma_f32_32x32x16_f16(fa[sb][pr == 1 ? 1 : 0][i], fb[sb][pr == 0 ? 1 : 0][j], acc[i][j], 0, 0, 0);
                            else acc[i][j] = __builtin_amdgcn_mfma_f32_32x32x16_bf16(fa[sb][pr == 1 ? 1 : 0][i], fb[sb][pr == 0 ? 1 : 0][j], acc[i][j], 0, 0, 0);
                        }
                        else acc[i][j][0] += (float)fa[sb][pr == 1 ? 1 : 0][i][0] * (float)fb[sb][pr == 0 ? 1 : 0][j][0];
                if (sb == 0 && ABL != 1 && more) issue_loads_part(buf ^ 1, pr);
                __builtin_amdgcn_sched_barrier(0);
            }
        __syncthreads();
    }
    flush(0);
}
#define IRSDE_WAIT_VM(N) asm volatile("s_waitcnt vmcnt(" #N ")" ::: "memory")
#define IRSDE_PHASE_BARRIER()                              \
    do {                                                   \
        asm volatile("s_waitcnt lgkmcnt(0)" ::: "memory"); \
        __builtin_amdgcn_s_barrier();                      \
    } while (0)
template <int ABL = 0, bool WALK = true, bool DRAIN = false>
__global__ __launch_bounds__(512, 1) void gemm_split3i_kernel(const SplitGemmArgs g) {
    constexpr int TM = 2, TN = 2, WN = 2, BM = 256, BN = 128;
    constexpr int ROWB = 192, GROUP = 16 * ROWB;
    constexpr int A_STAGE = BM * ROWB, STAGE = (BM + BN) * ROWB;
    constexpr int PA[6] = {0, 1, 2, 0, 1, 0};
    constexpr int PB[6] = {2, 1, 0, 1, 0, 0};
    extern __shared__ __attribute__((aligned(16))) char lds[];
    const int tid = threadIdx.x, lane = tid & 63;
    const int wave = __builtin_amdgcn_readfirstlane(tid >> 6);
    const int wm = wave / WN, wn = wave % WN;
    const int l31 = lane & 31, h = lane >> 5;
    const int mtiles = (g.M + BM - 1) / BM;
    const int units = mtiles * g.n_inner;
    const int xcd = blockIdx.x & 7, jx = blockIdx.x >> 3;
    const int ulo = (int)((long long)xcd * units / 8), uhi = (int)((long long)(xcd + 1) * units / 8);
    const int nitems = (uhi - ulo) * g.nblk_n;
    const int it_step = WALK ? ((int)gridDim.x - xcd + 7) >> 3 : nitems;
    int it = jx;
    if (it >= nitems) return;
    const int nk = g.K / SG_BK;
    const unsigned pairb = (unsigned)nk * 384u;

    const int ga0 = 4 * (wave >> 1) + (wave & 1);
    int plane0, m0, n0;
    unsigned a_voff[6], b_voff[3];
    const char *acomp, *bcomp;
    auto set_item = [&](int i) {
        const int unit = ulo + i / g.nblk_n, nblk = i % g.nblk_n;
        plane0 = unit / mtiles;
        m0 = (unit - plane0 * mtiles) * BM;
        n0 = nblk * BN;
#pragma unroll
        for (int q = 0; q < 9; ++q) {
            const int gi = q / 3, wl = q - gi * 3;
            const int sl = wl * 64 + lane;
            const int r = sl / 12, pos = sl - r * 12;
            int j = pos - ((r >> 2) & 3);
            j = j < 0 ? j + 12 : j;
            if (gi < 2) {
                int m = m0 + (ga0 + 2 * gi) * 16 + r;
                m = m < g.M ? m : g.M - 1;
                a_voff[q] = (unsigned)(m >> 1) * pairb + (unsigned)(m & 1) * 192u + (unsigned)j * 16u;
            } else {
                int n = n0 + wave * 16 + r;
                n = n < g.N ? n : g.N - 1;
                b_voff[wl] = (unsigned)(n >> 1) * pairb + (unsigned)(n & 1) * 192u + (unsigned)j * 16u;
            }
        }
        acomp = reinterpret_cast<const char*>(g.a) + (long long)plane0 * g.pA * 2;
        bcomp = reinterpret_cast<const char*>(g.b) + (long long)plane0 * g.pB * 2;
    };
    auto issue_unit = [&](int kb, int kind) {
        const char* gsrc = (kind < 2 ? acomp : bcomp) + (size_t)kb * 384;
        char* l = lds + (kb & 1) * STAGE + (kind < 2 ? (ga0 + 2 * kind) * GROUP : A_STAGE + wave * GROUP);
#pragma unroll
        for (int wl = 0; wl < 3; ++wl) IRSDE_GLDS16(gsrc + (kind < 2 ? a_voff[kind * 3 + wl] : b_voff[wl]), l + wl * 1024);
    };
    auto issue_one = [&](int kb, int kind, int wl) {
        const char* gsrc = (kind < 2 ? acomp : bcomp) + (size_t)kb * 384;
        char* l = lds + (kb & 1) * STAGE + (kind < 2 ? (ga0 + 2 * kind) * GROUP : A_STAGE + wave * GROUP);
        IRSDE_GLDS16(gsrc + (kind < 2 ? a_voff[kind * 3 + wl] : b_voff[wl]), l + wl * 1024);
    };
    auto issue_first = [&]() {
        issue_unit(0, 0);
        issue_unit(0, 2);
        issue_unit(0, 1);
        if (nk > 1) {
            issue_unit(1, 0);
            issue_unit(1, 2);
        }
    };

    floatx16 acc[TM][TN];
#pragma unroll
    for (int i = 0; i < TM; ++i)
#pragma unroll
        for (int j = 0; j < TN; ++j)
#pragma unroll
            for (int r = 0; r < 16; ++r) acc[i][j][r] = 0.f;

    set_item(it);
    issue_first();

    int fr_off[3][2];
#pragma unroll
    for (int p = 0; p < 3; ++p)
#pragma unroll
        for (int sb = 0; sb < 2; ++sb) fr_off[p][sb] = l31 * ROWB + ((p * 4 + sb * 2 + h + ((l31 >> 2) & 3)) % 12) * 16;
    bf16x8 fa[2][3], fb[2][3][TN];
    auto read_a = [&](int sb, const char* a) {
#pragma unroll
        for (int p = 0; p < 3; ++p) fa[sb][p] = *reinterpret_cast<const bf16x8*>(a + fr_off[p][sb]);
    };
    auto read_b = [&](int sb, const char* b) {
#pragma unroll
        for (int p = 0; p < 3; ++p)
#pragma unroll
            for (int j = 0; j < TN; ++j) fb[sb][p][j] = *reinterpret_cast<const bf16x8*>(b + j * 32 * ROWB + fr_off[p][sb]);
    };
    const bool late = wave >= 4;
    const int a_base = wm * TM * 32 * ROWB, b_base = A_STAGE + wn * TN * 32 * ROWB;
    for (;;) {
        IRSDE_WAIT_VM(0);
        IRSDE_PHASE_BARRIER();
        read_a(0, lds + a_base);
        read_b(0, lds + b_base);
        __builtin_amdgcn_sched_barrier(0);
        for (int st = 0; st < nk; ++st) {
            const bool more1 = st + 1 < nk, more2 = st + 2 < nk;
            const char* a = lds + (st & 1) * STAGE + a_base;
            const char* b = lds + (st & 1) * STAGE + b_base;
            const char* an = lds + ((st + 1) & 1) * STAGE + a_base;
            const char* bn = lds + ((st + 1) & 1) * STAGE + b_base;
#pragma unroll
            for (int i = 0; i < TM; ++i) {
                if (i == 1) {
                    read_a(0, a + 32 * ROWB);
                    __builtin_amdgcn_sched_barrier(0);
                }
#pragma unroll
                for (int sb = 0; sb < 2; ++sb)
#pragma unroll
                    for (int pr = 0; pr < 6; ++pr) {
#pragma unroll
                        for (int j = 0; j < TN; ++j) {
                            if (ABL != 3) acc[i][j] = __builtin_amdgcn_mfma_f32_32x32x16_bf16(fa[sb][PA[pr]], fb[sb][PB[pr]][j], acc[i][j], 0, 0, 0);
                            else acc[i][j][0] += (float)fa[sb][PA[pr]][0] * (float)fb[sb][PB[pr]][j][0];
                        }
                        __builtin_amdgcn_sched_barrier(0);
                        if (sb == 0 && pr == 0) {
                            if (i == 0) {
                                read_a(1, a);
                                read_b(1, b);
                            } else {
                                read_a(1, a + 32 * ROWB);
                            }
                        }
                        if (i == 1 && sb == 1 && pr == 0 && more1) {
                            read_a(0, an);
                            read_b(0, bn);
                        }
                        if (ABL != 1 && (sb == 1) == late) {
                            if (i == 0 && pr >= 1 && pr <= 3 && more1) issue_one(st + 1, 1, pr - 1);
                            if (i == 1 && more2) issue_one(st + 2, pr < 3 ? 0 : 2, pr % 3);
                        }
                        __builtin_amdgcn_sched_barrier(0);
                    }
                if (DRAIN || (i == 0 && !more1)) IRSDE_WAIT_VM(0);
                else if (i == 0) IRSDE_WAIT_VM(3);
                IRSDE_PHASE_BARRIER();
            }
        }

        const int rowb_ = m0 + wm * TM * 32, colb = n0 + wn * TN * 32;
        float* ob = g.out + (long long)plane0 * g.pO + (long long)rowb_ * g.ldc;
        const int rows = g.M - rowb_;
        const unsigned nrec = rows <= 0 ? 0u : (unsigned)(rows < TM * 32 ? rows : TM * 32) * (unsigned)g.ldc * 4u;
        const __amdgpu_buffer_rsrc_t ro = __builtin_amdgcn_make_buffer_rsrc(ob, 0, nrec, 0x00020000);
        it += it_step;
        const bool next = WALK && it < nitems;
        if (next) {
            set_item(it);
            issue_first();
            __builtin_amdgcn_sched_barrier(0);
        }
#pragma unroll
        for (int i = 0; i < TM; ++i)
#pragma unroll
            for (int j = 0; j < TN; ++j) {
                const int colu = colb + j * 32;
                if (colu + l31 < g.N && (ABL != 4 || acc[i][j][0] == 1.2345e30f)) {
#pragma unroll
                    for (int r = 0; r < 16; ++r) {
                        const float v = acc[i][j][r];
                        const unsigned voff = (unsigned)((i * 32 + (r & 3) + 8 * (r >> 2) + 4 * h) * g.ldc + colu + l31) * 4u;
                        __builtin_amdgcn_raw_buffer_store_b32(__builtin_bit_cast(unsigned, v), ro, (int)voff, 0, 0);
                    }
                }
            }
        if (!next) break;
#pragma unroll
        for (int i = 0; i < TM; ++i)
#pragma unroll
            for (int j = 0; j < TN; ++j)
#pragma unroll
                for (int r = 0; r < 16; ++r) acc[i][j][r] = 0.f;
    }
}
#undef IRSDE_PHASE_BARRIER
#undef IRSDE_WAIT_VM
#undef IRSDE_GLDS16

__global__ __launch_bounds__(256) void split_triples_kernel(const float* __restrict__ in, unsigned short* __restrict__ out, const size_t n, const size_t rows,
                                                            const int K) {
    const size_t i = (size_t)blockIdx.x * blockDim.x + threadIdx.x;
    if (i >= n) return;
    const size_t rk = rows * (size_t)K;
    const size_t z = i / rk, rem = i - z * rk;
    const size_t row = rem / K;
    const int k = (int)(rem - row * K);
    float r = in[i];
    unsigned short* o = out + z * split3_comp_elems(rows, K);
#pragma unroll
    for (int p = 0; p < 3; ++p) {
        const __bf16 hb = (__bf16)r;
        o[split3_index(row, k, p, K / 32)] = __builtin_bit_cast(unsigned short, hb);
        r -= (float)hb;
    }
}

template <bool F16>
__global__ __launch_bounds__(256) void split_pairs_kernel(const float* __restrict__ in, unsigned short* __restrict__ out, const size_t n, const int K,
                                                          const float scale) {
    const size_t i = (size_t)blockIdx.x * blockDim.x + threadIdx.x;
    if (i >= n) return;
    const size_t row = i / K;
    const int k = (int)(i - row * K);
    float r = in[i];
    const size_t base = (row * (size_t)(K / 32) + k / 32) * 64 + (k & 31);
    if constexpr (F16) {
        r *= scale;
        const _Float16 hb = (_Float16)r;
        out[base] = __builtin_bit_cast(unsigned short, hb);
        r -= (float)hb;
        const _Float16 lb = (_Float16)r;
        out[base + 32] = __builtin_bit_cast(unsigned short, lb);
    } else {
        const __bf16 hb = (__bf16)r;
        out[base] = __builtin_bit_cast(unsigned short, hb);
        r -= (float)hb;
        const __bf16 lb = (__bf16)r;
        out[base + 32] = __builtin_bit_cast(unsigned short, lb);
    }
}

template <int NPL, bool F16 = false>
__global__ __launch_bounds__(256) void split_planes_kernel(const float* __restrict__ in, unsigned short* __restrict__ out, const size_t n,
                                                           const size_t plane, const float scale) {
    const size_t i = (size_t)blockIdx.x * blockDim.x + threadIdx.x;
    if (i >= n) return;
    float r = F16 ? in[i] * scale : in[i];
#pragma unroll
    for (int p = 0; p < NPL; ++p) {
        if constexpr (F16) {
            const _Float16 hb = (_Float16)r;
            out[p * plane + i] = __builtin_bit_cast(unsigned short, hb);
            r -= (float)hb;
        } else {
            const __bf16 hb = (__bf16)r;
            out[p * plane + i] = __builtin_bit_cast(unsigned short, hb);
            r -= (float)hb;
        }
    }
}

}

void gemm_split_global_init() {
    IRSDE_HIP_CHECK(hipFuncSetAttribute(reinterpret_cast<const void*>(gemm_split2i_kernel<0>), hipFuncAttributeMaxDynamicSharedMemorySize, 160 * 1024));
    IRSDE_HIP_CHECK(hipFuncSetAttribute(reinterpret_cast<const void*>(gemm_split2i_kernel<0, true>), hipFuncAttributeMaxDynamicSharedMemorySize, 160 * 1024));
    IRSDE_HIP_CHECK(hipFuncSetAttribute(reinterpret_cast<const void*>(gemm_split2i_kernel<5, true>), hipFuncAttributeMaxDynamicSharedMemorySize, 160 * 1024));
    IRSDE_HIP_CHECK(hipFuncSetAttribute(reinterpret_cast<const void*>(gemm_split2i_kernel<1>), hipFuncAttributeMaxDynamicSharedMemorySize, 160 * 1024));
    IRSDE_HIP_CHECK(hipFuncSetAttribute(reinterpret_cast<const void*>(gemm_split2i_kernel<3>), hipFuncAttributeMaxDynamicSharedMemorySize, 160 * 1024));
    IRSDE_HIP_CHECK(hipFuncSetAttribute(reinterpret_cast<const void*>(gemm_split2i_kernel<4>), hipFuncAttributeMaxDynamicSharedMemorySize, 160 * 1024));
    IRSDE_HIP_CHECK(hipFuncSetAttribute(reinterpret_cast<const void*>(gemm_split3i_kernel<0, true>), hipFuncAttributeMaxDynamicSharedMemorySize, 160 * 1024));
    IRSDE_HIP_CHECK(hipFuncSetAttribute(reinterpret_cast<const void*>(gemm_split3i_kernel<0, false>), hipFuncAttributeMaxDynamicSharedMemorySize, 160 * 1024));
    IRSDE_HIP_CHECK(hipFuncSetAttribute(reinterpret_cast<const void*>(gemm_split3i_kernel<0, true, true>), hipFuncAttributeMaxDynamicSharedMemorySize, 160 * 1024));
#ifdef IRSDE_PROBES
    IRSDE_HIP_CHECK(hipFuncSetAttribute(reinterpret_cast<const void*>(gemm_split3i_kernel<1, true>), hipFuncAttributeMaxDynamicSharedMemorySize, 160 * 1024));
    IRSDE_HIP_CHECK(hipFuncSetAttribute(reinterpret_cast<const void*>(gemm_split3i_kernel<3, true>), hipFuncAttributeMaxDynamicSharedMemorySize, 160 * 1024));
    IRSDE_HIP_CHECK(hipFuncSetAttribute(reinterpret_cast<const void*>(gemm_split3i_kernel<4, true>), hipFuncAttributeMaxDynamicSharedMemorySize, 160 * 1024));
    IRSDE_HIP_CHECK(hipFuncSetAttribute(reinterpret_cast<const void*>(gemm_split3i_kernel<1, false>), hipFuncAttributeMaxDynamicSharedMemorySize, 160 * 1024));
    IRSDE_HIP_CHECK(hipFuncSetAttribute(reinterpret_cast<const void*>(gemm_split3i_kernel<3, false>), hipFuncAttributeMaxDynamicSharedMemorySize, 160 * 1024));
    IRSDE_HIP_CHECK(hipFuncSetAttribute(reinterpret_cast<const void*>(gemm_split3i_kernel<4, false>), hipFuncAttributeMaxDynamicSharedMemorySize, 160 * 1024));
    IRSDE_HIP_CHECK(hipFuncSetAttribute(reinterpret_cast<const void*>(gemm_split3i_kernel<1, true, true>), hipFuncAttributeMaxDynamicSharedMemorySize, 160 * 1024));
    IRSDE_HIP_CHECK(hipFuncSetAttribute(reinterpret_cast<const void*>(gemm_split3i_kernel<3, true, true>), hipFuncAttributeMaxDynamicSharedMemorySize, 160 * 1024));
    IRSDE_HIP_CHECK(hipFuncSetAttribute(reinterpret_cast<const void*>(gemm_split3i_kernel<4, true, true>), hipFuncAttributeMaxDynamicSharedMemorySize, 160 * 1024));
#endif
}

void launch_gemm_split_pairs(const SplitGemmArgs& a, int ncomp, hipStream_t s, int abl, bool f16) {
    if (a.K % SG_BK) throw HipError("gemm_split_pairs: K must be a multiple of 32");
    if ((unsigned long long)a.M * a.K * 4ull >= 0xffffffffull || (unsigned long long)a.N * a.K * 4ull >= 0xffffffffull ||
        (size_t)a.M * a.ldc * 4 >= 0xffffffffull)
        throw HipError("gemm_split_pairs: a component exceeds the 32-bit offset range");
    SplitGemmArgs g = a;
    g.nblk_n = (a.N + 255) / 256;
    g.n_inner = ncomp;
    const int units = ((a.M + 255) / 256) * ncomp;
    int per_xcd = 0;
    for (int x = 0; x < 8; ++x) per_xcd = std::max(per_xcd, (int)((long long)(x + 1) * units / 8) - (int)((long long)x * units / 8));
    const dim3 grid((unsigned)(8 * per_xcd * g.nblk_n));
    const size_t lds = (size_t)2 * 512 * 128;
    if (f16) {
        if (abl != 0) throw HipError("gemm_split_pairs: the ablation twins exist for the bf16 kernel only");
        static const bool nt = tuning_env_int("IRSDE_SPLIT_NT", 0) != 0;
        if (nt) hipLaunchKernelGGL((gemm_split2i_kernel<5, true>), grid, dim3(512), lds, s, g);
        else hipLaunchKernelGGL((gemm_split2i_kernel<0, true>), grid, dim3(512), lds, s, g);
        IRSDE_HIP_CHECK(hipGetLastError());
        return;
    }
    switch (abl) {
        case 0: hipLaunchKernelGGL(gemm_split2i_kernel<0>, grid, dim3(512), lds, s, g); break;
        case 1: hipLaunchKernelGGL(gemm_split2i_kernel<1>, grid, dim3(512), lds, s, g); break;
        case 3: hipLaunchKernelGGL(gemm_split2i_kernel<3>, grid, dim3(512), lds, s, g); break;
        case 4: hipLaunchKernelGGL(gemm_split2i_kernel<4>, grid, dim3(512), lds, s, g); break;
        default: throw HipError("gemm_split_pairs: bad ablation variant");
    }
    IRSDE_HIP_CHECK(hipGetLastError());
}

bool gemm_split_triples_fits(long long M, long long N, long long K, long long ldc) {
    if (M < 1 || N < 1 || K < 32 || K % SG_BK) return false;
    return (unsigned long long)split3_comp_elems((size_t)M, (size_t)K) * 2ull < 0xffffffffull && (unsigned long long)split3_comp_elems((size_t)N, (size_t)K) * 2ull < 0xffffffffull &&
           (unsigned long long)M * ldc * 4ull < 0xffffffffull;
}

static std::atomic<int> g_force_split3_blocks{-1};
void set_force_split3_blocks(int n) { g_force_split3_blocks.store(n >= 8 ? n : -1, std::memory_order_relaxed); }

template <int ABL>
static void launch_split3_abl(bool walk, bool drain, dim3 grid, size_t lds, hipStream_t s, const SplitGemmArgs& g) {
    if (drain) hipLaunchKernelGGL((gemm_split3i_kernel<ABL, true, true>), grid, dim3(512), lds, s, g);
    else if (walk) hipLaunchKernelGGL((gemm_split3i_kernel<ABL, true>), grid, dim3(512), lds, s, g);
    else hipLaunchKernelGGL((gemm_split3i_kernel<ABL, false>), grid, dim3(512), lds, s, g);
}
void launch_gemm_split_triples(const SplitGemmArgs& a, int ncomp, hipStream_t s, const Split3Launch& o) {
    if (a.K % SG_BK) throw HipError("gemm_split_triples: K must be a multiple of 32");
    if (!gemm_split_triples_fits(a.M, a.N, a.K, a.ldc)) throw HipError("gemm_split_triples: a component exceeds the 32-bit offset range");
    if (ncomp < 1 || a.ldc < a.N) throw HipError("gemm_split_triples: bad component count or output stride");
    static const bool walk_knob = tuning_env_int("IRSDE_SPLIT3_WALK", 1) != 0, drain_knob = tuning_env_int("IRSDE_SPLIT3_DRAIN", 0) != 0;
    const bool walk = o.walk == Split3Launch::RULE ? walk_knob : o.walk == Split3Launch::ON;
    const bool drain = o.drain == Split3Launch::RULE ? drain_knob : o.drain == Split3Launch::ON;
    if (drain && !walk) throw HipError("gemm_split_triples: the drain twin exists on the walk only");
    SplitGemmArgs g = a;
    g.nblk_n = (a.N + 127) / 128;
    g.n_inner = ncomp;
    const long long units = (long long)((a.M + 255) / 256) * ncomp;
    long long per_xcd = 0;
    for (int x = 0; x < 8; ++x) per_xcd = std::max(per_xcd, (x + 1) * units / 8 - x * units / 8);
    long long blocks = 8 * per_xcd * g.nblk_n;
    if (blocks >= 0x7fffffffll) throw HipError("gemm_split_triples: grid too large");
    if (walk) {
        const int forced = g_force_split3_blocks.load(std::memory_order_relaxed);
        blocks = std::min<long long>(blocks, std::max(8, forced > 0 ? forced : device_cu_count()));
    }
    const dim3 grid((unsigned)blocks);
    const size_t lds = (size_t)2 * (256 + 128) * 192;
    switch (o.abl) {
        case Split3Launch::FULL: launch_split3_abl<0>(walk, drain, grid, lds, s, g); break;
#ifdef IRSDE_PROBES
        case Split3Launch::NO_LOADS: launch_split3_abl<1>(walk, drain, grid, lds, s, g); break;
        case Split3Launch::NO_MFMA: launch_split3_abl<3>(walk, drain, grid, lds, s, g); break;
        case Split3Launch::NO_STORES: launch_split3_abl<4>(walk, drain, grid, lds, s, g); break;
#endif
        default: throw HipError("gemm_split_triples: the ablation twins are part of the PROBES build");
    }
    IRSDE_HIP_CHECK(hipGetLastError());
}

void launch_split_triples(const float* in, unsigned short* out, int ncomp, size_t rows, int K, hipStream_t s) {
    if (K % 32 || ncomp < 1 || rows < 1) throw HipError("split_triples: K must be a multiple of 32");
    const size_t n = (size_t)ncomp * rows * (size_t)K;
    hipLaunchKernelGGL(split_triples_kernel, dim3((unsigned)((n + 255) / 256)), dim3(256), 0, s, in, out, n, rows, K);
    IRSDE_HIP_CHECK(hipGetLastError());
}

void launch_split_pairs(const float* in, unsigned short* out, size_t rows, int K, hipStream_t s, bool f16, float scale) {
    if (K % 32) throw HipError("split_pairs: K must be a multiple of 32");
    const size_t n = rows * (size_t)K;
    if (f16) hipLaunchKernelGGL(split_pairs_kernel<true>, dim3((unsigned)((n + 255) / 256)), dim3(256), 0, s, in, out, n, K, scale);
    else hipLaunchKernelGGL(split_pairs_kernel<false>, dim3((unsigned)((n + 255) / 256)), dim3(256), 0, s, in, out, n, K, 1.0f);
    IRSDE_HIP_CHECK(hipGetLastError());
}

void launch_split_planes(const float* in, unsigned short* out, size_t n, size_t plane, int nplanes, hipStream_t s, bool f16, float scale) {
    const dim3 grid((unsigned)((n + 255) / 256));
    if (f16 && nplanes != 2) throw HipError("split_planes: fp16 pieces come in pairs");
    if (f16) hipLaunchKernelGGL((split_planes_kernel<2, true>), grid, dim3(256), 0, s, in, out, n, plane, scale);
    else if (nplanes == 2) hipLaunchKernelGGL((split_planes_kernel<2, false>), grid, dim3(256), 0, s, in, out, n, plane, 1.0f);
    else throw HipError("split_planes: 2 planes");
    IRSDE_HIP_CHECK(hipGetLastError());
}

}
```

### image_restoration_sde_amd/csrc/split3_layout.h

```cpp
#pragma once
#include <cstddef>

namespace irsde {

#if defined(__HIPCC__) || defined(__CUDACC__)
#define IRSDE_S3_HD __host__ __device__
#else
#define IRSDE_S3_HD
#endif

IRSDE_S3_HD inline size_t split3_rows(size_t rows) { return (rows + 1) & ~(size_t)1; }
IRSDE_S3_HD inline size_t split3_comp_elems(size_t rows, size_t K) { return split3_rows(rows) * K * 3; }
IRSDE_S3_HD inline size_t split3_index(size_t row, size_t k, int p, size_t nkb) {
    return ((row >> 1) * nkb + (k >> 5)) * 192 + (row & 1) * 96 + (size_t)p * 32 + (k & 31);
}

#undef IRSDE_S3_HD

}
```

### include/irsde_hip_debug.h

```cpp
#ifndef IRSDE_HIP_DEBUG_H
#define IRSDE_HIP_DEBUG_H

#include "irsde_hip.h"

#ifdef __cplusplus
extern "C" {
#endif

int irsde_debug_conv(const float* in0, int C0, const float* in1, int C1, int B, int Hin, int Win, int in_shift,
                     const float* w_oihw, int Cout, int KH, int KW, int stride, int pad, const float* bias,
                     const float* film, int film_bstride, int silu, const float* res, float* out, int naive,
                     int splits, void* stream);

int irsde_debug_conv_choice(int B, int Hin, int Win, int C0, int C1, int Cout, int K, int stride, int pad, int in_shift, int operand, int storage, int pair,
                            unsigned features, int splits, int nz, int tune, int cu_count, const int* knobs, char* out, int out_len);

int irsde_debug_conv_features(const float* in0, int C0, const float* in1, int C1, int B, int Hin, int Win, int in_shift, const float* w_oihw, int Cout, int K,
                              int stride, int pad, int operand, int storage, int pair, const float* bias, const float* ch_scale, const float* ln_g,
                              const float* film, int film_bstride, const float* res, const float* in_scale, const float* gate_film, int gate_film_bstride,
                              int silu, int gate, int shuffle, int nz, int splits, int tune, const int* knobs, float* out, char* choice, int choice_len,
                              void* stream);

int irsde_debug_split_gemm(const float* A, const float* B, float* C, int M, int N, int K, int ncomp, int nplanes, void* stream);

int irsde_bench_conv(int variant, int B, int H, int W, int Cin, int Cout, int K, int stride, int up, int epi, int iters,
                     double* ms_out);
int irsde_bench_naf_chain(int variant, int nblocks, int B, int iters, double* ms_out);
int irsde_debug_force_subbatches(int n);
int irsde_debug_force_chain_groups(int g);
int irsde_debug_force_wino_poly(int mode);
int irsde_debug_force_split3(int mode);
int irsde_debug_force_split3_blocks(int n);

int irsde_debug_scam(const float* x, int B_pairs, int H, int W, int C, const float* norm_l_g, const float* norm_r_g, const float* l_proj1_w,
                     const float* l_proj1_b, const float* r_proj1_w, const float* r_proj1_b, const float* l_proj2_w, const float* l_proj2_b,
                     const float* r_proj2_w, const float* r_proj2_b, const float* beta, const float* gamma, float* out, void* stream);

int irsde_debug_naf_gate_sca(const float* u, int B, int H, int W, int c, const float* conv2_w, const float* conv2_b, const float* sca_w, const float* sca_b,
                             float* gated_out, float* mean_out, float* s_out, void* stream);
int irsde_debug_tlsc(const float* g, int B, int h, int w, int c, int k1, int k2, float* pooled_out, const float* scale_map, float* scaled_out, void* stream);
int irsde_debug_ln_film(const float* x, long long M, int C, long long ppi, const float* g, const float* fscale, const float* fshift, int film_bstride,
                        float* out, void* stream);
int irsde_debug_naf_lnconv(int mode, const float* x, long long M, int c, int Cout, long long ppi, const float* g, const float* fscale, const float* fshift,
                           int film_bstride, const float* w, const float* bias, const float* gate_film, int gate_film_bstride, const float* in_scale,
                           const float* ch_scale, const float* res, float* out, void* stream);

int irsde_debug_naf_chain(const float* x, float* out, int B, int nblocks, const float* norm1_g, const float* conv1_w, const float* conv1_b, const float* conv2_w,
                          const float* conv2_b, const float* sca_w, const float* sca_b, const float* conv3_w, const float* conv3_b, const float* beta,
                          const float* norm2_g, const float* conv4_w, const float* conv4_b, const float* conv5_w, const float* conv5_b, const float* gamma,
                          const float* film, int film_bstride, int film_off, const float* cam, int cam_bstride, int cam_off, int groups, void* stream);
int irsde_debug_naf_chain_split_order(int nblocks, int groups, int* order_out, long long n);

int irsde_debug_full_attention16(const void* qkv_bf16, int B, int N, void* out_bf16, void* stream);

int irsde_debug_scam_full(const float* x, int B_pairs, int H, int W, int C, const float* norm_l_g, const float* norm_r_g, const float* l_proj1_w,
                          const float* l_proj1_b, const float* r_proj1_w, const float* r_proj1_b, const float* l_proj2_w, const float* l_proj2_b,
                          const float* r_proj2_w, const float* r_proj2_b, const float* beta, const float* gamma, float* out, void* stream);

int irsde_debug_scam_stream(const float* x, int B_pairs, int H, int W, int C, const float* norm_l_g, const float* norm_r_g, const float* l_proj1_w,
                            const float* l_proj1_b, const float* r_proj1_w, const float* r_proj1_b, const float* l_proj2_w, const float* l_proj2_b,
                            const float* r_proj2_w, const float* r_proj2_b, const float* beta, const float* gamma, int block_w, float* out, void* stream);
int irsde_debug_scam_full_stream(const float* x, int B_pairs, int H, int W, int C, const float* norm_l_g, const float* norm_r_g, const float* l_proj1_w,
                                 const float* l_proj1_b, const float* r_proj1_w, const float* r_proj1_b, const float* l_proj2_w, const float* l_proj2_b,
                                 const float* r_proj2_w, const float* r_proj2_b, const float* beta, const float* gamma, int block_w, float* out,
                                 void* stream);
int irsde_debug_force_scam_stream(int block_w);

#ifdef __cplusplus
}
#endif
#endif
```

Measured before the change: 4.630 images/s.

## Split split3 GEMM tail items into halves and prefetch across item seams

Adds two features to the persistent split-triple bf16 GEMM kernel, both on by default. 'Halves' splits the leftover tail items of each XCD's work ring into half-M items so the last wave of items is spread over twice as many blocks. 'Seam' lets the double-buffered LDS ring start prefetching the next item's K-slices during the last stages of the current item, so the pipeline does not drain at each item boundary. Both aim to cut tail imbalance and per-item pipeline bubbles, at the cost of more template variants, extra registers and more complex control flow that could hurt scheduling.

Result: no change. 4.649 images/s, median of 6 (+0.4%).

```diff
diff --git a/image_restoration_sde_amd/_lib.py b/image_restoration_sde_amd/_lib.py
--- a/image_restoration_sde_amd/_lib.py
+++ b/image_restoration_sde_amd/_lib.py
@@ -39,7 +39,7 @@
     "irsde_last_error", "irsde_version", "irsde_create", "irsde_create_nafnet", "irsde_destroy", "irsde_num_weights",
     "irsde_weight_name", "irsde_weight_shape", "irsde_load_weight", "irsde_finalize_weights",
     "irsde_set_schedule", "irsde_unet_forward", "irsde_sample", "irsde_sde_step", "irsde_philox_normal",
-    "irsde_get_profile", "irsde_debug_tap", "irsde_work_model", "irsde_debug_conv", "irsde_debug_conv_choice", "irsde_debug_conv_features", "irsde_plan_describe", "irsde_bench_conv", "irsde_op_profile", "irsde_debug_split_gemm", "irsde_bench_naf_chain", "irsde_debug_force_subbatches", "irsde_debug_force_chain_groups", "irsde_debug_force_wino_poly", "irsde_debug_force_split3", "irsde_debug_force_split3_blocks", "irsde_debug_scam", "irsde_debug_scam_full",
+    "irsde_get_profile", "irsde_debug_tap", "irsde_work_model", "irsde_debug_conv", "irsde_debug_conv_choice", "irsde_debug_conv_features", "irsde_plan_describe", "irsde_bench_conv", "irsde_op_profile", "irsde_debug_split_gemm", "irsde_bench_naf_chain", "irsde_debug_force_subbatches", "irsde_debug_force_chain_groups", "irsde_debug_force_wino_poly", "irsde_debug_force_split3", "irsde_debug_force_split3_blocks", "irsde_debug_split3_deal", "irsde_debug_scam", "irsde_debug_scam_full",
     "irsde_debug_scam_stream", "irsde_debug_scam_full_stream", "irsde_debug_force_scam_stream",
     "irsde_debug_naf_gate_sca", "irsde_debug_tlsc", "irsde_debug_ln_film", "irsde_debug_naf_lnconv", "irsde_debug_naf_chain", "irsde_debug_naf_chain_split_order",
     "irsde_debug_full_attention16",
@@ -132,6 +132,7 @@
     lib.irsde_debug_force_wino_poly.argtypes = [c.c_int]
     lib.irsde_debug_force_split3.argtypes = [c.c_int]
     lib.irsde_debug_force_split3_blocks.argtypes = [c.c_int]
+    lib.irsde_debug_split3_deal.argtypes = [c.c_int] * 5 + [c.POINTER(c.c_int), c.c_int64, c.POINTER(c.c_int64)]
     lib.irsde_debug_scam.argtypes = [P, c.c_int, c.c_int, c.c_int, c.c_int] + [P] * 12 + [P, P]
     lib.irsde_debug_scam_full.argtypes = [P, c.c_int, c.c_int, c.c_int, c.c_int] + [P] * 12 + [P, P]
     lib.irsde_debug_scam_stream.argtypes = [P, c.c_int, c.c_int, c.c_int, c.c_int] + [P] * 12 + [c.c_int, P, P]
diff --git a/image_restoration_sde_amd/csrc/common.h b/image_restoration_sde_amd/csrc/common.h
--- a/image_restoration_sde_amd/csrc/common.h
+++ b/image_restoration_sde_amd/csrc/common.h
@@ -136,8 +136,15 @@
     Abl abl = FULL;
     Tri walk = RULE;
     Tri drain = RULE;
+    Tri halves = RULE;
+    Tri seam = RULE;
 };
 void launch_gemm_split_triples(const SplitGemmArgs& a, int ncomp, hipStream_t s, const Split3Launch& o = {});
+struct Split3Deal {
+    long long item;
+    int half;
+};
+std::vector<std::vector<Split3Deal>> split3_deal(int M, int N, int ncomp, int blocks, bool halves);
 void set_force_split3_blocks(int n);
 bool gemm_split_triples_fits(long long M, long long N, long long K, long long ldc);
 void launch_split_triples(const float* in, unsigned short* out, int ncomp, size_t rows, int K, hipStream_t s);
diff --git a/image_restoration_sde_amd/csrc/engine_debug.hip b/image_restoration_sde_amd/csrc/engine_debug.hip
--- a/image_restoration_sde_amd/csrc/engine_debug.hip
+++ b/image_restoration_sde_amd/csrc/engine_debug.hip
@@ -88,7 +88,9 @@
     Split3Launch o;
     o.abl = static_cast<Split3Launch::Abl>(abl);
     o.walk = twin == 0 ? Split3Launch::RULE : twin == 1 ? Split3Launch::OFF : Split3Launch::ON;
-    o.drain = twin == 0 ? Split3Launch::RULE : twin == 1 ? Split3Launch::OFF : Split3Launch::ON;
+    o.drain = twin == 0 ? Split3Launch::RULE : twin == 2 ? Split3Launch::ON : Split3Launch::OFF;
+    o.halves = twin == 0 ? Split3Launch::RULE : twin == 4 || twin == 6 ? Split3Launch::ON : Split3Launch::OFF;
+    o.seam = twin == 0 ? Split3Launch::RULE : twin == 5 || twin == 6 ? Split3Launch::ON : Split3Launch::OFF;
     return o;
 }
 
@@ -195,7 +197,7 @@
     bench(465, 465, BenchKind::Fused64TStamps, 5),
     bench(4650, 4653, BenchKind::Fused64TStamps, 12),
     bench(472, 476, BenchKind::PairGemm, 0),
-    bench(490, 504, BenchKind::TripleGemm, 0),
+    bench(490, 524, BenchKind::TripleGemm, 0),
 };
 
 template <class Row, size_t N, class Lo, class Hi>
@@ -884,8 +886,8 @@
 
 int irsde_debug_split_gemm(const float* A, const float* Bm, float* C, int M, int N, int K, int ncomp, int nplanes, void* stream) {
     return guard([&] {
-        const int twin3 = nplanes == 43 ? 0 : nplanes == 45 ? 1 : nplanes == 47 ? 2 : -1;
-        if (twin3 < 0 && nplanes != 42 && nplanes != 44) throw HipError("debug_split_gemm: nplanes must be 42, 43, 44, 45 or 47");
+        const int twin3 = nplanes == 43 ? 0 : nplanes == 45 ? 1 : nplanes == 47 ? 2 : nplanes == 50 ? 3 : nplanes == 49 ? 4 : nplanes == 51 ? 5 : nplanes == 52 ? 6 : -1;
+        if (twin3 < 0 && nplanes != 42 && nplanes != 44) throw HipError("debug_split_gemm: nplanes must be 42, 43, 44, 45, 47 or 49 .. 52");
         hipStream_t s = reinterpret_cast<hipStream_t>(stream);
         conv_global_init();
         Scratch mem(s);
@@ -914,6 +916,24 @@
     if (n >= 0 && n < 8) return guard([&] { throw HipError("debug_force_split3_blocks: n must be at least 8 (one block per XCD), or negative for the default"); });
     set_force_split3_blocks(n);
     return IRSDE_OK;
+}
+
+int irsde_debug_split3_deal(int M, int N, int ncomp, int blocks, int halves, int* out, long long cap, long long* n_out) {
+    return guard([&] {
+        if (!out || !n_out || cap < 0) throw HipError("debug_split3_deal: bad argument");
+        const std::vector<std::vector<Split3Deal>> deal = split3_deal(M, N, ncomp, blocks, halves != 0);
+        long long n = 0;
+        for (const auto& d : deal) n += (long long)d.size();
+        *n_out = n;
+        if (n > cap) throw HipError("debug_split3_deal: the deal has " + std::to_string(n) + " entries");
+        for (size_t b = 0; b < deal.size(); ++b)
+            for (const Split3Deal& d : deal[b]) {
+                if (d.item > 0x7fffffffll) throw HipError("debug_split3_deal: item number out of range");
+                *out++ = (int)b;
+                *out++ = (int)d.item;
+                *out++ = d.half;
+            }
+    });
 }
 
 int irsde_debug_force_wino_poly(int mode) {
diff --git a/image_restoration_sde_amd/csrc/gemm_split.hip b/image_restoration_sde_amd/csrc/gemm_split.hip
--- a/image_restoration_sde_amd/csrc/gemm_split.hip
+++ b/image_restoration_sde_amd/csrc/gemm_split.hip
@@ -2,6 +2,7 @@
 #include <algorithm>
 #include <atomic>
 #include <type_traits>
+#include <vector>
 
 namespace irsde {
 
@@ -173,8 +174,10 @@
         asm volatile("s_waitcnt lgkmcnt(0)" ::: "memory"); \
         __builtin_amdgcn_s_barrier();                      \
     } while (0)
-template <int ABL = 0, bool WALK = true, bool DRAIN = false>
+template <int ABL = 0, bool WALK = true, bool DRAIN = false, bool HALVES = false, bool SEAM = false>
 __global__ __launch_bounds__(512, 1) void gemm_split3i_kernel(const SplitGemmArgs g) {
+    static_assert(!HALVES || WALK, "half items exist on the walk only");
+    static_assert(!SEAM || (WALK && !DRAIN), "the ring crosses item seams on the walk's ring only");
     constexpr int TM = 2, TN = 2, WN = 2, BM = 256, BN = 128;
     constexpr int ROWB = 192, GROUP = 16 * ROWB;
     constexpr int A_STAGE = BM * ROWB, STAGE = (BM + BN) * ROWB;
@@ -192,7 +195,14 @@
     const int nitems = (uhi - ulo) * g.nblk_n;
     const int it_step = WALK ? ((int)gridDim.x - xcd + 7) >> 3 : nitems;
     int it = jx;
-    if (it >= nitems) return;
+    int nfull = nitems, hcode = -1;
+    if constexpr (HALVES) {
+        const int rem = split3_half_items(nitems, it_step);
+        nfull = nitems - rem;
+        if (jx < 2 * rem) hcode = 2 * nfull + jx;
+    }
+    const bool have_full = !HALVES || it < nfull;
+    if (HALVES ? !have_full && hcode < 0 : it >= nitems) return;
     const int nk = g.K / SG_BK;
     const unsigned pairb = (unsigned)nk * 384u;
 
@@ -200,7 +210,9 @@
     int plane0, m0, n0;
     unsigned a_voff[6], b_voff[3];
     const char *acomp, *bcomp;
-    auto set_item = [&](int i) {
+    int plane0n = 0, m0n = 0, n0n = 0, par = 0;
+    const char *acomp_n = nullptr, *bcomp_n = nullptr;
+    auto set_offsets = [&](int i, int units, int& plane0, int& m0, int& n0) {
         const int unit = ulo + i / g.nblk_n, nblk = i % g.nblk_n;
         plane0 = unit / mtiles;
         m0 = (unit - plane0 * mtiles) * BM;
@@ -208,6 +220,7 @@
 #pragma unroll
         for (int q = 0; q < 9; ++q) {
             const int gi = q / 3, wl = q - gi * 3;
+            if (!((units >> gi) & 1)) continue;
             const int sl = wl * 64 + lane;
             const int r = sl / 12, pos = sl - r * 12;
             int j = pos - ((r >> 2) & 3);
@@ -222,20 +235,24 @@
                 b_voff[wl] = (unsigned)(n >> 1) * pairb + (unsigned)(n & 1) * 192u + (unsigned)j * 16u;
             }
         }
+    };
+    auto set_item = [&](int i) {
+        set_offsets(i, 7, plane0, m0, n0);
         acomp = reinterpret_cast<const char*>(g.a) + (long long)plane0 * g.pA * 2;
         bcomp = reinterpret_cast<const char*>(g.b) + (long long)plane0 * g.pB * 2;
     };
+    auto stage_of = [&](int kb) { return SEAM ? (kb + par) & 1 : kb & 1; };
     auto issue_unit = [&](int kb, int kind) {
         const char* gsrc = (kind < 2 ? acomp : bcomp) + (size_t)kb * 384;
-        char* l = lds + (kb & 1) * STAGE + (kind < 2 ? (ga0 + 2 * kind) * GROUP : A_STAGE + wave * GROUP);
+        char* l = lds + stage_of(kb) * STAGE + (kind < 2 ? (ga0 + 2 * kind) * GROUP : A_STAGE + wave * GROUP);
 #pragma unroll
         for (int wl = 0; wl < 3; ++wl) IRSDE_GLDS16(gsrc + (kind < 2 ? a_voff[kind * 3 + wl] : b_voff[wl]), l + wl * 1024);
     };
-    auto issue_one = [&](int kb, int kind, int wl) {
-        const char* gsrc = (kind < 2 ? acomp : bcomp) + (size_t)kb * 384;
-        char* l = lds + (kb & 1) * STAGE + (kind < 2 ? (ga0 + 2 * kind) * GROUP : A_STAGE + wave * GROUP);
+    auto issue_one_at = [&](int stage, const char* gsrc, int kind, int wl) {
+        char* l = lds + stage * STAGE + (kind < 2 ? (ga0 + 2 * kind) * GROUP : A_STAGE + wave * GROUP);
         IRSDE_GLDS16(gsrc + (kind < 2 ? a_voff[kind * 3 + wl] : b_voff[wl]), l + wl * 1024);
     };
+    auto issue_one = [&](int kb, int kind, int wl) { issue_one_at(stage_of(kb), (kind < 2 ? acomp : bcomp) + (size_t)kb * 384, kind, wl); };
     auto issue_first = [&]() {
         issue_unit(0, 0);
         issue_unit(0, 2);
@@ -254,8 +271,32 @@
 #pragma unroll
             for (int r = 0; r < 16; ++r) acc[i][j][r] = 0.f;
 
-    set_item(it);
-    issue_first();
+    constexpr int HSTAGE = 16 * GROUP;
+    auto issue_half_one = [&](int kb, int q) {
+        const char* gsrc = (q < 3 ? acomp : bcomp) + (size_t)kb * 384;
+        char* l = lds + (kb % 3) * HSTAGE + ((q < 3 ? 0 : 8) + wave) * GROUP;
+        IRSDE_GLDS16(gsrc + (q < 3 ? a_voff[q] : b_voff[q - 3]), l + (q % 3) * 1024);
+    };
+    auto open_half = [&]() {
+        int hc = hcode;
+        asm volatile("" : "+s"(hc));
+        set_item(hc >> 1);
+        if (hc & 1) {
+#pragma unroll
+            for (int wl = 0; wl < 3; ++wl) a_voff[wl] = a_voff[3 + wl];
+        }
+#pragma unroll
+        for (int kb = 0; kb < 3; ++kb)
+            if (kb < nk) {
+#pragma unroll
+                for (int q = 0; q < 6; ++q) issue_half_one(kb, q);
+            }
+    };
+
+    if (have_full) {
+        set_item(it);
+        issue_first();
+    }
 
     int fr_off[3][2];
 #pragma unroll
@@ -275,18 +316,31 @@
     };
     const bool late = wave >= 4;
     const int a_base = wm * TM * 32 * ROWB, b_base = A_STAGE + wn * TN * 32 * ROWB;
-    for (;;) {
+    if (have_full) for (;;) {
         IRSDE_WAIT_VM(0);
         IRSDE_PHASE_BARRIER();
-        read_a(0, lds + a_base);
-        read_b(0, lds + b_base);
+        read_a(0, lds + stage_of(0) * STAGE + a_base);
+        read_b(0, lds + stage_of(0) * STAGE + b_base);
         __builtin_amdgcn_sched_barrier(0);
+        const bool tail = SEAM && nk >= 3 && it + it_step < nfull;
         for (int st = 0; st < nk; ++st) {
             const bool more1 = st + 1 < nk, more2 = st + 2 < nk;
-            const char* a = lds + (st & 1) * STAGE + a_base;
-            const char* b = lds + (st & 1) * STAGE + b_base;
-            const char* an = lds + ((st + 1) & 1) * STAGE + a_base;
-            const char* bn = lds + ((st + 1) & 1) * STAGE + b_base;
+            const bool go1 = more1 || tail, go2 = more2 || tail;
+            if constexpr (SEAM) {
+                if (tail && st == nk - 2) {
+                    set_offsets(it + it_step, 5, plane0n, m0n, n0n);
+                    acomp_n = reinterpret_cast<const char*>(g.a) + (long long)plane0n * g.pA * 2;
+                    bcomp_n = reinterpret_cast<const char*>(g.b) + (long long)plane0n * g.pB * 2;
+                }
+                if (tail && st == nk - 1) set_offsets(it + it_step, 2, plane0n, m0n, n0n);
+            }
+            const char* src_a1 = (more1 ? acomp : acomp_n) + (size_t)(more1 ? st + 1 : st + 1 - nk) * 384;
+            const char* src_a2 = (more2 ? acomp : acomp_n) + (size_t)(more2 ? st + 2 : st + 2 - nk) * 384;
+            const char* src_b2 = (more2 ? bcomp : bcomp_n) + (size_t)(more2 ? st + 2 : st + 2 - nk) * 384;
+            const char* a = lds + stage_of(st) * STAGE + a_base;
+            const char* b = lds + stage_of(st) * STAGE + b_base;
+            const char* an = lds + stage_of(st + 1) * STAGE + a_base;
+            const char* bn = lds + stage_of(st + 1) * STAGE + b_base;
 #pragma unroll
             for (int i = 0; i < TM; ++i) {
                 if (i == 1) {
@@ -316,12 +370,17 @@
                             read_b(0, bn);
                         }
                         if (ABL != 1 && (sb == 1) == late) {
-                            if (i == 0 && pr >= 1 && pr <= 3 && more1) issue_one(st + 1, 1, pr - 1);
-                            if (i == 1 && more2) issue_one(st + 2, pr < 3 ? 0 : 2, pr % 3);
+                            if constexpr (SEAM) {
+                                if (i == 0 && pr >= 1 && pr <= 3 && go1) issue_one_at(stage_of(st + 1), src_a1, 1, pr - 1);
+                                if (i == 1 && go2) issue_one_at(stage_of(st), pr < 3 ? src_a2 : src_b2, pr < 3 ? 0 : 2, pr % 3);
+                            } else {
+                                if (i == 0 && pr >= 1 && pr <= 3 && more1) issue_one(st + 1, 1, pr - 1);
+                                if (i == 1 && more2) issue_one(st + 2, pr < 3 ? 0 : 2, pr % 3);
+                            }
                         }
                         __builtin_amdgcn_sched_barrier(0);
                     }
-                if (DRAIN || (i == 0 && !more1)) IRSDE_WAIT_VM(0);
+                if (DRAIN || (i == 0 && !go1)) IRSDE_WAIT_VM(0);
                 else if (i == 0) IRSDE_WAIT_VM(3);
                 IRSDE_PHASE_BARRIER();
             }
@@ -333,10 +392,17 @@
         const unsigned nrec = rows <= 0 ? 0u : (unsigned)(rows < TM * 32 ? rows : TM * 32) * (unsigned)g.ldc * 4u;
         const __amdgpu_buffer_rsrc_t ro = __builtin_amdgcn_make_buffer_rsrc(ob, 0, nrec, 0x00020000);
         it += it_step;
-        const bool next = WALK && it < nitems;
-        if (next) {
+        const bool next = WALK && it < nfull;
+        if constexpr (SEAM) par = (par + nk) & 1;
+        if (SEAM && tail) {
+            plane0 = plane0n, m0 = m0n, n0 = n0n;
+            acomp = acomp_n, bcomp = bcomp_n;
+        } else if (next) {
             set_item(it);
             issue_first();
+            __builtin_amdgcn_sched_barrier(0);
+        } else if (HALVES && hcode >= 0) {
+            open_half();
             __builtin_amdgcn_sched_barrier(0);
         }
 #pragma unroll
@@ -360,6 +426,94 @@
             for (int j = 0; j < TN; ++j)
 #pragma unroll
                 for (int r = 0; r < 16; ++r) acc[i][j][r] = 0.f;
+    }
+
+    if constexpr (HALVES) {
+        if (hcode < 0) return;
+        const int hh = hcode & 1;
+        if (have_full) {
+#pragma unroll
+            for (int j = 0; j < TN; ++j)
+#pragma unroll
+                for (int r = 0; r < 16; ++r) acc[0][j][r] = 0.f;
+        } else {
+            open_half();
+        }
+        int hl = lane;
+        asm volatile("" : "+v"(hl));
+        int hfr[3][2];
+#pragma unroll
+        for (int p = 0; p < 3; ++p)
+#pragma unroll
+            for (int sb = 0; sb < 2; ++sb) hfr[p][sb] = (hl & 31) * ROWB + ((p * 4 + sb * 2 + (hl >> 5) + (((hl & 31) >> 2) & 3)) % 12) * 16;
+        auto read_a = [&](int sb, const char* a) {
+#pragma unroll
+            for (int p = 0; p < 3; ++p) fa[sb][p] = *reinterpret_cast<const bf16x8*>(a + hfr[p][sb]);
+        };
+        auto read_b = [&](int sb, const char* b) {
+#pragma unroll
+            for (int p = 0; p < 3; ++p)
+#pragma unroll
+                for (int j = 0; j < TN; ++j) fb[sb][p][j] = *reinterpret_cast<const bf16x8*>(b + j * 32 * ROWB + hfr[p][sb]);
+        };
+        const int ha_base = wm * 32 * ROWB, hb_base = 8 * GROUP + wn * TN * 32 * ROWB;
+        IRSDE_WAIT_VM(0);
+        IRSDE_PHASE_BARRIER();
+        read_a(0, lds + ha_base);
+        read_b(0, lds + hb_base);
+        __builtin_amdgcn_sched_barrier(0);
+        for (int st = 0; st < nk; ++st) {
+            const bool more1 = st + 1 < nk, more2 = st + 2 < nk, more3 = st + 3 < nk;
+            const char* cur = lds + (st % 3) * HSTAGE;
+            const char* nxt = lds + ((st + 1) % 3) * HSTAGE;
+#pragma unroll
+            for (int sb = 0; sb < 2; ++sb)
+#pragma unroll
+                for (int pr = 0; pr < 6; ++pr) {
+#pragma unroll
+                    for (int j = 0; j < TN; ++j) {
+                        if (ABL != 3) acc[0][j] = __builtin_amdgcn_mfma_f32_32x32x16_bf16(fa[sb][PA[pr]], fb[sb][PB[pr]][j], acc[0][j], 0, 0, 0);
+                        else acc[0][j][0] += (float)fa[sb][PA[pr]][0] * (float)fb[sb][PB[pr]][j][0];
+                    }
+                    __builtin_amdgcn_sched_barrier(0);
+                    if (sb == 0 && pr == 0) {
+                        read_a(1, cur + ha_base);
+                        read_b(1, cur + hb_base);
+                    }
+                    if (sb == 1 && pr == 0 && more1) {
+                        read_a(0, nxt + ha_base);
+                        read_b(0, nxt + hb_base);
+                    }
+                    if (ABL != 1) {
+                        if (sb == 1 && !late && more3) issue_half_one(st + 3, pr);
+                        if (sb == 0 && late && st >= 1 && more2) issue_half_one(st + 2, pr);
+                    }
+                    __builtin_amdgcn_sched_barrier(0);
+                    if (sb == 0 && pr == 5) {
+                        if (DRAIN || !more2) IRSDE_WAIT_VM(0);
+                        else IRSDE_WAIT_VM(6);
+                        IRSDE_PHASE_BARRIER();
+                        __builtin_amdgcn_sched_barrier(0);
+                    }
+                }
+        }
+        const int rowb_ = m0 + wm * TM * 32 + hh * 32, colb = n0 + wn * TN * 32;
+        float* ob = g.out + (long long)plane0 * g.pO + (long long)rowb_ * g.ldc;
+        const int rows = g.M - rowb_;
+        const unsigned nrec = rows <= 0 ? 0u : (unsigned)(rows < 32 ? rows : 32) * (unsigned)g.ldc * 4u;
+        const __amdgpu_buffer_rsrc_t ro = __builtin_amdgcn_make_buffer_rsrc(ob, 0, nrec, 0x00020000);
+#pragma unroll
+        for (int j = 0; j < TN; ++j) {
+            const int colu = colb + j * 32;
+            if (colu + l31 < g.N && (ABL != 4 || acc[0][j][0] == 1.2345e30f)) {
+#pragma unroll
+                for (int r = 0; r < 16; ++r) {
+                    const unsigned voff = (unsigned)(((r & 3) + 8 * (r >> 2) + 4 * h) * g.ldc + colu + l31) * 4u;
+                    const float v = acc[0][j][r];
+                    __builtin_amdgcn_raw_buffer_store_b32(__builtin_bit_cast(unsigned, v), ro, (int)voff, 0, 0);
+                }
+            }
+        }
     }
 }
 #undef IRSDE_PHASE_BARRIER
@@ -431,6 +585,12 @@
 
 }
 
+template <int ABL>
+static void split3_features_init() {
+    IRSDE_HIP_CHECK(hipFuncSetAttribute(reinterpret_cast<const void*>(gemm_split3i_kernel<ABL, true, false, true, false>), hipFuncAttributeMaxDynamicSharedMemorySize, 160 * 1024));
+    IRSDE_HIP_CHECK(hipFuncSetAttribute(reinterpret_cast<const void*>(gemm_split3i_kernel<ABL, true, false, false, true>), hipFuncAttributeMaxDynamicSharedMemorySize, 160 * 1024));
+    IRSDE_HIP_CHECK(hipFuncSetAttribute(reinterpret_cast<const void*>(gemm_split3i_kernel<ABL, true, false, true, true>), hipFuncAttributeMaxDynamicSharedMemorySize, 160 * 1024));
+}
 void gemm_split_global_init() {
     IRSDE_HIP_CHECK(hipFuncSetAttribute(reinterpret_cast<const void*>(gemm_split2i_kernel<0>), hipFuncAttributeMaxDynamicSharedMemorySize, 160 * 1024));
     IRSDE_HIP_CHECK(hipFuncSetAttribute(reinterpret_cast<const void*>(gemm_split2i_kernel<0, true>), hipFuncAttributeMaxDynamicSharedMemorySize, 160 * 1024));
@@ -441,7 +601,11 @@
     IRSDE_HIP_CHECK(hipFuncSetAttribute(reinterpret_cast<const void*>(gemm_split3i_kernel<0, true>), hipFuncAttributeMaxDynamicSharedMemorySize, 160 * 1024));
     IRSDE_HIP_CHECK(hipFuncSetAttribute(reinterpret_cast<const void*>(gemm_split3i_kernel<0, false>), hipFuncAttributeMaxDynamicSharedMemorySize, 160 * 1024));
     IRSDE_HIP_CHECK(hipFuncSetAttribute(reinterpret_cast<const void*>(gemm_split3i_kernel<0, true, true>), hipFuncAttributeMaxDynamicSharedMemorySize, 160 * 1024));
+    split3_features_init<0>();
 #ifdef IRSDE_PROBES
+    split3_features_init<1>();
+    split3_features_init<3>();
+    split3_features_init<4>();
     IRSDE_HIP_CHECK(hipFuncSetAttribute(reinterpret_cast<const void*>(gemm_split3i_kernel<1, true>), hipFuncAttributeMaxDynamicSharedMemorySize, 160 * 1024));
     IRSDE_HIP_CHECK(hipFuncSetAttribute(reinterpret_cast<const void*>(gemm_split3i_kernel<3, true>), hipFuncAttributeMaxDynamicSharedMemorySize, 160 * 1024));
     IRSDE_HIP_CHECK(hipFuncSetAttribute(reinterpret_cast<const void*>(gemm_split3i_kernel<4, true>), hipFuncAttributeMaxDynamicSharedMemorySize, 160 * 1024));
@@ -491,12 +655,41 @@
            (unsigned long long)M * ldc * 4ull < 0xffffffffull;
 }
 
+std::vector<std::vector<Split3Deal>> split3_deal(int M, int N, int ncomp, int blocks, bool halves) {
+    if (M < 1 || N < 1 || ncomp < 1 || blocks < 8) throw HipError("split3_deal: M, N, ncomp >= 1 and at least 8 blocks");
+    const int nblk_n = (N + 127) / 128;
+    const long long units = (long long)((M + 255) / 256) * ncomp;
+    std::vector<std::vector<Split3Deal>> deal((size_t)blocks);
+    for (int b = 0; b < blocks; ++b) {
+        const int xcd = b & 7, jx = b >> 3;
+        const long long ulo = xcd * units / 8, uhi = (xcd + 1) * units / 8;
+        const long long n = (uhi - ulo) * nblk_n, first = ulo * nblk_n;
+        const int nb = (blocks - xcd + 7) >> 3;
+        const int rem = halves && n < 0x7fffffffll ? split3_half_items((int)n, nb) : 0;
+        for (long long i = jx; i < n - rem; i += nb) deal[b].push_back({first + i, -1});
+        if (jx < 2 * rem) deal[b].push_back({first + n - rem + (jx >> 1), jx & 1});
+    }
+    return deal;
+}
+static bool split3_deals_halves(int M, int N, int ncomp, int blocks) {
+    const int nblk_n = (N + 127) / 128;
+    const long long units = (long long)((M + 255) / 256) * ncomp;
+    for (int xcd = 0; xcd < 8; ++xcd) {
+        const long long n = ((xcd + 1) * units / 8 - xcd * units / 8) * nblk_n;
+        if (n > 0 && n < 0x7fffffffll && split3_half_items((int)n, (blocks - xcd + 7) >> 3) > 0) return true;
+    }
+    return false;
+}
+
 static std::atomic<int> g_force_split3_blocks{-1};
 void set_force_split3_blocks(int n) { g_force_split3_blocks.store(n >= 8 ? n : -1, std::memory_order_relaxed); }
 
 template <int ABL>
-static void launch_split3_abl(bool walk, bool drain, dim3 grid, size_t lds, hipStream_t s, const SplitGemmArgs& g) {
-    if (drain) hipLaunchKernelGGL((gemm_split3i_kernel<ABL, true, true>), grid, dim3(512), lds, s, g);
+static void launch_split3_abl(bool walk, bool drain, bool halves, bool seam, dim3 grid, size_t lds, hipStream_t s, const SplitGemmArgs& g) {
+    if (halves && seam) hipLaunchKernelGGL((gemm_split3i_kernel<ABL, true, false, true, true>), grid, dim3(512), lds, s, g);
+    else if (seam) hipLaunchKernelGGL((gemm_split3i_kernel<ABL, true, false, false, true>), grid, dim3(512), lds, s, g);
+    else if (halves) hipLaunchKernelGGL((gemm_split3i_kernel<ABL, true, false, true>), grid, dim3(512), lds, s, g);
+    else if (drain) hipLaunchKernelGGL((gemm_split3i_kernel<ABL, true, true>), grid, dim3(512), lds, s, g);
     else if (walk) hipLaunchKernelGGL((gemm_split3i_kernel<ABL, true>), grid, dim3(512), lds, s, g);
     else hipLaunchKernelGGL((gemm_split3i_kernel<ABL, false>), grid, dim3(512), lds, s, g);
 }
@@ -508,6 +701,12 @@
     const bool walk = o.walk == Split3Launch::RULE ? walk_knob : o.walk == Split3Launch::ON;
     const bool drain = o.drain == Split3Launch::RULE ? drain_knob : o.drain == Split3Launch::ON;
     if (drain && !walk) throw HipError("gemm_split_triples: the drain twin exists on the walk only");
+    static const bool halves_knob = tuning_env_int("IRSDE_SPLIT3_HALVES", 1) != 0;
+    bool halves = o.halves == Split3Launch::RULE ? halves_knob && walk && !drain : o.halves == Split3Launch::ON;
+    if (halves && (!walk || drain)) throw HipError("gemm_split_triples: half items exist on the walk's ring only");
+    static const bool seam_knob = tuning_env_int("IRSDE_SPLIT3_SEAM", 1) != 0;
+    const bool seam = o.seam == Split3Launch::RULE ? seam_knob && walk && !drain : o.seam == Split3Launch::ON;
+    if (seam && (!walk || drain)) throw HipError("gemm_split_triples: the ring crosses item seams on the walk's ring only");
     SplitGemmArgs g = a;
     g.nblk_n = (a.N + 127) / 128;
     g.n_inner = ncomp;
@@ -522,12 +721,13 @@
     }
     const dim3 grid((unsigned)blocks);
     const size_t lds = (size_t)2 * (256 + 128) * 192;
+    if (halves && !split3_deals_halves(a.M, a.N, ncomp, (int)blocks)) halves = false;
     switch (o.abl) {
-        case Split3Launch::FULL: launch_split3_abl<0>(walk, drain, grid, lds, s, g); break;
+        case Split3Launch::FULL: launch_split3_abl<0>(walk, drain, halves, seam, grid, lds, s, g); break;
 #ifdef IRSDE_PROBES
-        case Split3Launch::NO_LOADS: launch_split3_abl<1>(walk, drain, grid, lds, s, g); break;
-        case Split3Launch::NO_MFMA: launch_split3_abl<3>(walk, drain, grid, lds, s, g); break;
-        case Split3Launch::NO_STORES: launch_split3_abl<4>(walk, drain, grid, lds, s, g); break;
+        case Split3Launch::NO_LOADS: launch_split3_abl<1>(walk, drain, halves, seam, grid, lds, s, g); break;
+        case Split3Launch::NO_MFMA: launch_split3_abl<3>(walk, drain, halves, seam, grid, lds, s, g); break;
+        case Split3Launch::NO_STORES: launch_split3_abl<4>(walk, drain, halves, seam, grid, lds, s, g); break;
 #endif
         default: throw HipError("gemm_split_triples: the ablation twins are part of the PROBES build");
     }
diff --git a/image_restoration_sde_amd/csrc/split3_layout.h b/image_restoration_sde_amd/csrc/split3_layout.h
--- a/image_restoration_sde_amd/csrc/split3_layout.h
+++ b/image_restoration_sde_amd/csrc/split3_layout.h
@@ -15,6 +15,11 @@
     return ((row >> 1) * nkb + (k >> 5)) * 192 + (row & 1) * 96 + (size_t)p * 32 + (k & 31);
 }
 
+IRSDE_S3_HD inline int split3_half_items(int nitems, int nb) {
+    const int rem = nitems % nb;
+    return rem > 0 && 2 * rem <= nb ? rem : 0;
+}
+
 #undef IRSDE_S3_HD
 
 }
diff --git a/include/irsde_hip_debug.h b/include/irsde_hip_debug.h
--- a/include/irsde_hip_debug.h
+++ b/include/irsde_hip_debug.h
@@ -31,6 +31,7 @@
 int irsde_debug_force_wino_poly(int mode);
 int irsde_debug_force_split3(int mode);
 int irsde_debug_force_split3_blocks(int n);
+int irsde_debug_split3_deal(int M, int N, int ncomp, int blocks, int halves, int* out, long long cap, long long* n_out);
 
 int irsde_debug_scam(const float* x, int B_pairs, int H, int W, int C, const float* norm_l_g, const float* norm_r_g, const float* l_proj1_w,
                      const float* l_proj1_b, const float* r_proj1_w, const float* r_proj1_b, const float* l_proj2_w, const float* l_proj2_b,
```
